# anshumang/gunrockINST

Measured on AMD Instinct MI355X. Metric: MTEPS (million traversed edges/sec) BFS R-MAT scale-24, higher is better.
Workload: dtype int32; 1 GPU; BFS idempotent direction-optimizing (traversal_mode 2), R-MAT scale-24 (a=.55 b=.2 c=.2 d=.05, 8 pairs/vertex mirrored, seed 0x6772): n=16777216, m=265395436 directed edges; sources: largest-degree + 64 seeded; search_depth_src0=7, max_degree=218420

## Files before the change

gunrockinst_amd/capi.py:

```python
import ctypes as C
import os
import subprocess

import numpy as np

_PKG = os.path.dirname(os.path.abspath(__file__))
LIB_PATH = os.environ.get("GUNROCK_LIB_PATH") or os.path.join(_PKG, "lib", "libgunrock.so")
_LIB = None

VTXID_INT = 0
SIZET_INT = 0
VALUE_INT, VALUE_UINT, VALUE_FLOAT = 0, 1, 2
SRC_MANUALLY, SRC_RANDOMIZE, SRC_LARGEST_DEGREE = 0, 1, 2

i32p = C.POINTER(C.c_int32)


class GunrockDataType(C.Structure):
    _fields_ = [("VTXID_TYPE", C.c_int), ("SIZET_TYPE", C.c_int), ("VALUE_TYPE", C.c_int)]


class GunrockGraph(C.Structure):
    _fields_ = [("num_nodes", C.c_size_t), ("num_edges", C.c_size_t),
                ("row_offsets", C.c_void_p), ("col_indices", C.c_void_p),
                ("col_offsets", C.c_void_p), ("row_indices", C.c_void_p),
                ("node_values", C.c_void_p), ("edge_values", C.c_void_p)]


class GunrockConfig(C.Structure):
    _fields_ = [("mark_pred", C.c_bool), ("idempotence", C.c_bool),
                ("src_node", C.c_int), ("device", C.c_int), ("max_iter", C.c_int),
                ("top_nodes", C.c_int), ("delta_factor", C.c_int),
                ("delta", C.c_float), ("error", C.c_float), ("queue_size", C.c_float),
                ("src_mode", C.c_int)]


def build_library(force=False):
    src_dir = os.path.join(_PKG, "csrc")
    if force:
        subprocess.check_call(["make", "-C", src_dir, "clean"])
    subprocess.check_call(["make", "-C", src_dir, "-j8", "-s"])
    return LIB_PATH


_SIGNATURES = {
    "gunrock_bfs_func": (None, [C.POINTER(GunrockGraph), C.POINTER(GunrockGraph), GunrockConfig, GunrockDataType]),
    "gunrock_bc_func": (None, [C.POINTER(GunrockGraph), C.POINTER(GunrockGraph), GunrockConfig, GunrockDataType]),
    "gunrock_cc_func": (None, [C.POINTER(GunrockGraph), C.POINTER(GunrockGraph), GunrockConfig, GunrockDataType]),
    "gunrock_sssp_func": (None, [C.POINTER(GunrockGraph), C.c_void_p, C.POINTER(GunrockGraph), GunrockConfig,
                                 GunrockDataType]),
    "gunrock_pr_func": (None, [C.POINTER(GunrockGraph), C.c_void_p, C.c_void_p, C.POINTER(GunrockGraph),
                               GunrockConfig, GunrockDataType]),
    "gunrock_topk_func": (None, [C.POINTER(GunrockGraph), C.c_void_p, C.c_void_p, C.c_void_p,
                                 C.POINTER(GunrockGraph), GunrockConfig, GunrockDataType]),
    "grx_graph_from_market": (C.c_int, [C.c_char_p, C.c_int, C.c_int, C.POINTER(C.c_void_p)]),
    "grx_graph_from_market_cached": (C.c_int, [C.c_char_p, C.c_int, C.c_int, C.POINTER(C.c_int), C.POINTER(C.c_void_p)]),
    "grx_graph_rmat_libc": (C.c_int, [C.c_int, C.c_int, C.c_int] + [C.c_double] * 4 + [C.POINTER(C.c_void_p)]),
    "grx_graph_rmat_seeded": (C.c_int, [C.c_int, C.c_longlong, C.c_uint64, C.c_int] + [C.c_double] * 4 +
                              [C.POINTER(C.c_void_p)]),
    "grx_graph_from_coo": (C.c_int, [C.c_int, C.c_longlong, i32p, i32p, i32p, C.POINTER(C.c_void_p)]),
    "grx_graph_from_csr": (C.c_int, [C.c_int, C.c_int, i32p, i32p, i32p, C.POINTER(C.c_void_p)]),
    "grx_graph_nodes": (C.c_int, [C.c_void_p]),
    "grx_graph_edges": (C.c_int, [C.c_void_p]),
    "grx_graph_row_offsets": (i32p, [C.c_void_p]),
    "grx_graph_col_indices": (i32p, [C.c_void_p]),
    "grx_graph_edge_values": (i32p, [C.c_void_p]),
    "grx_graph_highest_degree_node": (C.c_int, [C.c_void_p, i32p]),
    "grx_graph_average_degree": (C.c_int, [C.c_void_p]),
    "grx_random_node": (C.c_int, [C.c_int]),
    "grx_graph_free": (None, [C.c_void_p]),
    "grx_rmat_seeded_device": (C.c_int, [C.c_int, C.c_longlong, C.c_longlong, C.c_uint64] + [C.c_double] * 4 +
                               [C.c_void_p, C.c_void_p, C.c_void_p]),
    "grx_coo_to_csr_sort": (C.c_int, [C.POINTER(C.c_void_p), C.c_int, C.c_int, C.c_longlong, C.c_void_p, C.c_void_p, C.c_int,
                                      C.c_int, C.c_int, C.POINTER(C.c_longlong), C.c_void_p]),
    "grx_coo_to_csr_emit": (C.c_int, [C.c_void_p, C.c_void_p, C.c_void_p, C.c_void_p]),
    "grx_coo_to_csr_free": (None, [C.c_void_p]),
    "grx_bc_create": (C.c_int, [C.POINTER(C.c_void_p), C.c_int]),
    "grx_bc_init": (C.c_int, [C.c_void_p, C.c_int, C.c_int, C.c_void_p, C.c_void_p]),
    "grx_bc_init_device": (C.c_int, [C.c_void_p, C.c_int, C.c_int, C.c_void_p, C.c_void_p]),
    "grx_bc_run": (C.c_int, [C.c_void_p, C.c_int, C.c_int, C.c_double, C.POINTER(C.c_float)]),
    "grx_bc_extract": (C.c_int, [C.c_void_p, C.c_void_p, C.c_void_p, C.c_void_p]),
    "grx_bc_destroy": (None, [C.c_void_p]),
    "grx_bfs_create": (C.c_int, [C.POINTER(C.c_void_p), C.c_int, C.c_int, C.c_int, C.c_int]),
    "grx_bfs_init": (C.c_int, [C.c_void_p, C.c_int, C.c_int, i32p, i32p]),
    "grx_bfs_init_device": (C.c_int, [C.c_void_p, C.c_int, C.c_int, C.c_void_p, C.c_void_p]),
    "grx_bfs_set_inverse_graph": (C.c_int, [C.c_void_p, C.c_void_p, C.c_void_p, C.c_float, C.c_float]),
    "grx_bfs_auto_inverse": (C.c_int, [C.c_void_p, C.c_int, C.POINTER(C.c_int), C.POINTER(C.c_int), C.POINTER(C.c_float)]),
    "grx_bfs_set_tuning": (C.c_int, [C.c_void_p, C.c_float, C.c_float, C.c_float, C.c_int]),
    "grx_bfs_set_persistent_limit": (C.c_int, [C.c_void_p, C.c_int]),
    "grx_bfs_set_twc_limit": (C.c_int, [C.c_void_p, C.c_int]),
    "grx_bfs_set_binned_min_edges": (C.c_int, [C.c_void_p, C.c_longlong]),
    "grx_bfs_set_label_deferral": (C.c_int, [C.c_void_p, C.c_int, C.c_int]),
    "grx_bfs_set_option": (C.c_int, [C.c_void_p, C.c_char_p, C.c_double]),
    "grx_bfs_set_cooperative_launch": (C.c_int, [C.c_void_p, C.c_int]),
    "grx_bfs_set_head_pass": (C.c_int, [C.c_void_p, C.c_int, C.c_int]),
    "grx_bfs_reset": (C.c_int, [C.c_void_p, C.c_int, C.c_double]),
    "grx_bfs_enact": (C.c_int, [C.c_void_p, C.c_int, C.c_int, C.c_int, C.POINTER(C.c_float)]),
    "grx_bfs_stats": (C.c_int, [C.c_void_p, C.POINTER(C.c_longlong), C.POINTER(C.c_longlong),
                                C.POINTER(C.c_double), C.POINTER(C.c_longlong), C.POINTER(C.c_double)]),
    "grx_bfs_level_trace": (C.c_int, [C.c_void_p, C.c_int, C.POINTER(C.c_longlong), C.POINTER(C.c_longlong),
                                      C.POINTER(C.c_double), i32p]),
    "grx_bfs_extract": (C.c_int, [C.c_void_p, i32p, i32p]),
    "grx_bfs_device_results": (C.c_int, [C.c_void_p, C.POINTER(C.c_void_p), C.POINTER(C.c_void_p)]),
    "grx_bfs_mask_flushes": (C.c_int, [C.c_void_p, C.POINTER(C.c_longlong)]),
    "grx_bfs_relabel_info": (C.c_int, [C.c_void_p, C.POINTER(C.c_longlong), C.POINTER(C.c_longlong), C.POINTER(C.c_int),
                                       C.POINTER(C.c_float), C.POINTER(C.c_longlong)]),
    "grx_bfs_destroy": (None, [C.c_void_p]),
    "grx_cc_create": (C.c_int, [C.POINTER(C.c_void_p), C.c_int, C.c_int]),
    "grx_cc_init": (C.c_int, [C.c_void_p, C.c_int, C.c_int, i32p, i32p]),
    "grx_cc_init_device": (C.c_int, [C.c_void_p, C.c_int, C.c_int, C.c_void_p, C.c_void_p]),
    "grx_cc_reset": (C.c_int, [C.c_void_p]),
    "grx_cc_enact": (C.c_int, [C.c_void_p, C.c_int, C.POINTER(C.c_float)]),
    "grx_cc_stats": (C.c_int, [C.c_void_p, C.POINTER(C.c_longlong), C.POINTER(C.c_longlong), C.POINTER(C.c_longlong),
                               C.POINTER(C.c_double)]),
    "grx_cc_mirrored": (C.c_int, [C.c_void_p, C.POINTER(C.c_int)]),
    "grx_cc_sweep_edges": (C.c_int, [C.c_void_p, C.POINTER(C.c_longlong)]),
    "grx_cc_extract": (C.c_int, [C.c_void_p, i32p, C.POINTER(C.c_uint)]),
    "grx_cc_device_results": (C.c_int, [C.c_void_p, C.POINTER(C.c_void_p)]),
    "grx_cc_destroy": (None, [C.c_void_p]),
    "grx_mst_create": (C.c_int, [C.POINTER(C.c_void_p), C.c_int, C.c_int]),
    "grx_mst_init": (C.c_int, [C.c_void_p, C.c_int, C.c_int, i32p, i32p, i32p]),
    "grx_mst_init_device": (C.c_int, [C.c_void_p, C.c_int, C.c_int, C.c_void_p, C.c_void_p, C.c_void_p]),
    "grx_mst_reset": (C.c_int, [C.c_void_p]),
    "grx_mst_enact": (C.c_int, [C.c_void_p, C.c_int, C.POINTER(C.c_float)]),
    "grx_mst_stats": (C.c_int, [C.c_void_p, C.POINTER(C.c_longlong), C.POINTER(C.c_longlong), C.POINTER(C.c_longlong),
                                C.POINTER(C.c_double)]),
    "grx_mst_round_trace": (C.c_int, [C.c_void_p, C.c_int, C.POINTER(C.c_longlong), C.POINTER(C.c_double)]),
    "grx_mst_extract": (C.c_int, [C.c_void_p, i32p, C.POINTER(C.c_longlong), C.POINTER(C.c_int)]),
    "grx_mst_device_results": (C.c_int, [C.c_void_p, C.POINTER(C.c_void_p)]),
    "grx_mst_destroy": (None, [C.c_void_p]),
    "grx_mis_create": (C.c_int, [C.POINTER(C.c_void_p), C.c_int, C.c_int]),
    "grx_mis_init": (C.c_int, [C.c_void_p, C.c_int, C.c_int, i32p, i32p, i32p, C.c_uint]),
    "grx_mis_init_device": (C.c_int, [C.c_void_p, C.c_int, C.c_int, C.c_void_p, C.c_void_p, C.c_void_p, C.c_uint]),
    "grx_mis_set_tail": (C.c_int, [C.c_void_p, C.c_int]),
    "grx_mis_reset": (C.c_int, [C.c_void_p]),
    "grx_mis_enact": (C.c_int, [C.c_void_p, C.c_int, C.c_int, C.POINTER(C.c_float)]),
    "grx_mis_stats": (C.c_int, [C.c_void_p, C.POINTER(C.c_longlong), C.POINTER(C.c_longlong), C.POINTER(C.c_longlong),
                                C.POINTER(C.c_longlong), C.POINTER(C.c_longlong), C.POINTER(C.c_double)]),
    "grx_mis_round_trace": (C.c_int, [C.c_void_p, C.c_int, C.POINTER(C.c_longlong), C.POINTER(C.c_double)]),
    "grx_mis_extract": (C.c_int, [C.c_void_p, i32p, C.POINTER(C.c_longlong)]),
    "grx_mis_device_results": (C.c_int, [C.c_void_p, C.POINTER(C.c_void_p)]),
    "grx_mis_destroy": (None, [C.c_void_p]),
    "grx_tc_create": (C.c_int, [C.POINTER(C.c_void_p), C.c_int, C.c_int]),
    "grx_tc_init": (C.c_int, [C.c_void_p, C.c_int, C.c_int, i32p, i32p]),
    "grx_tc_init_device": (C.c_int, [C.c_void_p, C.c_int, C.c_int, C.c_void_p, C.c_void_p]),
    "grx_tc_set_option": (C.c_int, [C.c_void_p, C.c_char_p, C.c_double]),
    "grx_tc_reset": (C.c_int, [C.c_void_p]),
    "grx_tc_enact": (C.c_int, [C.c_void_p, C.c_int, C.POINTER(C.c_float)]),
    "grx_tc_stats": (C.c_int, [C.c_void_p, C.POINTER(C.c_longlong), C.POINTER(C.c_longlong), C.POINTER(C.c_longlong),
                               C.POINTER(C.c_longlong), C.POINTER(C.c_longlong), C.POINTER(C.c_double), C.POINTER(C.c_double)]),
    "grx_tc_extract": (C.c_int, [C.c_void_p, C.POINTER(C.c_longlong), C.POINTER(C.c_longlong)]),
    "grx_tc_clustering": (C.c_int, [C.c_void_p, C.POINTER(C.c_double), C.POINTER(C.c_double)]),
    "grx_tc_device_results": (C.c_int, [C.c_void_p, C.POINTER(C.c_void_p), C.POINTER(C.c_void_p)]),
    "grx_tc_destroy": (None, [C.c_void_p]),
    "grx_kcore_create": (C.c_int, [C.POINTER(C.c_void_p), C.c_int, C.c_int]),
    "grx_kcore_init": (C.c_int, [C.c_void_p, C.c_int, C.c_int, i32p, i32p]),
    "grx_kcore_init_device": (C.c_int, [C.c_void_p, C.c_int, C.c_int, C.c_void_p, C.c_void_p]),
    "grx_kcore_set_option": (C.c_int, [C.c_void_p, C.c_char_p, C.c_double]),
    "grx_kcore_reset": (C.c_int, [C.c_void_p]),
    "grx_kcore_enact": (C.c_int, [C.c_void_p, C.c_int, C.c_int, C.POINTER(C.c_float)]),
    "grx_kcore_stats": (C.c_int, [C.c_void_p] + [C.POINTER(C.c_longlong)] * 8 + [C.POINTER(C.c_double)] * 2),
    "grx_kcore_level_trace": (C.c_int, [C.c_void_p, C.c_int, i32p, C.POINTER(C.c_longlong), C.POINTER(C.c_double)]),
    "grx_kcore_extract": (C.c_int, [C.c_void_p, i32p, C.POINTER(C.c_int)]),
    "grx_kcore_shells": (C.c_int, [C.c_void_p, C.c_int, C.POINTER(C.c_longlong)]),
    "grx_kcore_members": (C.c_int, [C.c_void_p, C.c_int, C.POINTER(C.c_ubyte), C.POINTER(C.c_longlong), C.POINTER(C.c_longlong)]),
    "grx_kcore_device_results": (C.c_int, [C.c_void_p, C.POINTER(C.c_void_p), C.POINTER(C.c_void_p)]),
    "grx_kcore_destroy": (None, [C.c_void_p]),
    "grx_truss_create": (C.c_int, [C.POINTER(C.c_void_p), C.c_int, C.c_int]),
    "grx_truss_init": (C.c_int, [C.c_void_p, C.c_int, C.c_int, i32p, i32p]),
    "grx_truss_init_device": (C.c_int, [C.c_void_p, C.c_int, C.c_int, C.c_void_p, C.c_void_p]),
    "grx_truss_set_option": (C.c_int, [C.c_void_p, C.c_char_p, C.c_double]),
    "grx_truss_reset": (C.c_int, [C.c_void_p]),
    "grx_truss_enact": (C.c_int, [C.c_void_p, C.c_int, C.c_int, C.POINTER(C.c_float)]),
    "grx_truss_stats": (C.c_int, [C.c_void_p] + [C.POINTER(C.c_longlong)] * 10 + [C.POINTER(C.c_double)] * 3),
    "grx_truss_level_trace": (C.c_int, [C.c_void_p, C.c_int, i32p, C.POINTER(C.c_longlong), C.POINTER(C.c_double)]),
    "grx_truss_edges": (C.c_int, [C.c_void_p, i32p, i32p]),
    "grx_truss_support": (C.c_int, [C.c_void_p, i32p, C.POINTER(C.c_longlong)]),
    "grx_truss_extract": (C.c_int, [C.c_void_p, i32p, C.POINTER(C.c_int)]),
    "grx_truss_classes": (C.c_int, [C.c_void_p, C.c_int, C.POINTER(C.c_longlong)]),
    "grx_truss_members": (C.c_int, [C.c_void_p, C.c_int, C.POINTER(C.c_ubyte), C.POINTER(C.c_longlong), C.POINTER(C.c_longlong)]),
    "grx_truss_vertex_truss": (C.c_int, [C.c_void_p, i32p]),
    "grx_truss_device_results": (C.c_int, [C.c_void_p] + [C.POINTER(C.c_void_p)] * 4),
    "grx_truss_destroy": (None, [C.c_void_p]),
    "grx_sssp_create": (C.c_int, [C.POINTER(C.c_void_p), C.c_int, C.c_int, C.c_int]),
    "grx_sssp_init": (C.c_int, [C.c_void_p, C.c_int, C.c_int, i32p, i32p, C.POINTER(C.c_uint32), C.c_int]),
    "grx_sssp_init_device": (C.c_int, [C.c_void_p, C.c_int, C.c_int, C.c_void_p, C.c_void_p, C.c_void_p, C.c_float]),
    "grx_sssp_set_inverse_graph": (C.c_int, [C.c_void_p, C.c_void_p, C.c_void_p, C.c_void_p, C.c_longlong]),
# ... 234 lines not shown

    def set_inverse_graph(self, d_inv_row_offsets=None, d_inv_col_indices=None, alpha=0.0, beta=0.0):
        _check(lib().grx_bfs_set_inverse_graph(self._h, C.c_void_p(d_inv_row_offsets), C.c_void_p(d_inv_col_indices),
                                               alpha, beta), "BFSProblem::SetInverseGraph")
        return self

    def auto_inverse(self, build_if_directed=True):
        on, made, ms = C.c_int(), C.c_int(), C.c_float()
        _check(lib().grx_bfs_auto_inverse(self._h, int(bool(build_if_directed)), C.byref(on), C.byref(made), C.byref(ms)),
               "grx_bfs_auto_inverse")
        return bool(on.value), bool(made.value), float(ms.value)

    def set_tuning(self, alpha=0.0, beta=0.0, lite_factor=-1.0, tail_edge_limit=-1):
        _check(lib().grx_bfs_set_tuning(self._h, alpha, beta, lite_factor, tail_edge_limit), "grx_bfs_set_tuning")
        return self

    def set_head_pass(self, min_edges=-1, max_edges=-1):
        _check(lib().grx_bfs_set_head_pass(self._h, int(min_edges), int(max_edges)), "grx_bfs_set_head_pass")
        return self

    def set_option(self, name, value):
        _check(lib().grx_bfs_set_option(self._h, name.encode(), float(value)), "grx_bfs_set_option(%s)" % name)
        return self

    def set_label_deferral(self, enabled=-1, mask_limit=0):
        _check(lib().grx_bfs_set_label_deferral(self._h, int(enabled), int(mask_limit)), "grx_bfs_set_label_deferral")
        return self

    def set_binned_min_edges(self, min_edges):
        _check(lib().grx_bfs_set_binned_min_edges(self._h, int(min_edges)), "grx_bfs_set_binned_min_edges")
        return self

    def set_cooperative_launch(self, on=True):
        _check(lib().grx_bfs_set_cooperative_launch(self._h, int(bool(on))), "grx_bfs_set_cooperative_launch")
        return self

    def set_persistent_limit(self, edge_limit):
        _check(lib().grx_bfs_set_persistent_limit(self._h, int(edge_limit)), "grx_bfs_set_persistent_limit")
        return self

    def set_twc_limit(self, edge_limit):
        _check(lib().grx_bfs_set_twc_limit(self._h, int(edge_limit)), "grx_bfs_set_twc_limit")
        return self

    def reset(self, src, queue_sizing=1.0):
        _check(lib().grx_bfs_reset(self._h, int(src), float(queue_sizing)), "BFSProblem::Reset")

    def enact(self, src, max_grid_size=0, traversal_mode=0):
        return self._timed(lib().grx_bfs_enact, "BFSEnactor::Enact", int(src), max_grid_size, traversal_mode)

    def stats(self):
        q, d, l = C.c_longlong(), C.c_longlong(), C.c_longlong()
        duty, kms = C.c_double(), C.c_double()
        _check(lib().grx_bfs_stats(self._h, C.byref(q), C.byref(d), C.byref(duty), C.byref(l), C.byref(kms)),
               "BFSEnactor::GetStatistics")
        return {"total_queued": q.value, "search_depth": d.value, "avg_duty": duty.value,
                "kernel_launches": l.value, "kernel_ms": kms.value}

    def level_trace(self, max_levels=4096):
        fr = (C.c_longlong * max_levels)()
        ed = (C.c_longlong * max_levels)()
        ms = (C.c_double * max_levels)()
        kd = (C.c_int32 * max_levels)()
        n = lib().grx_bfs_level_trace(self._h, max_levels, fr, ed, ms, kd)
        n = min(max(n, 0), max_levels)
        return [{"frontier": fr[i], "edges": ed[i], "ms": ms[i], "kind": kd[i]} for i in range(n)]

    def extract(self):
        labels = np.empty(max(self.nodes, 1), dtype=np.int32)
        preds = np.empty(max(self.nodes, 1), dtype=np.int32) if self.mark_pred else None
        _check(lib().grx_bfs_extract(self._h, _p(labels), None if preds is None else _p(preds)), "BFSProblem::Extract")
        return labels[:self.nodes], (None if preds is None else preds[:self.nodes])

    def device_results(self):
        dl, dp = C.c_void_p(), C.c_void_p()
        _check(lib().grx_bfs_device_results(self._h, C.byref(dl), C.byref(dp)), "grx_bfs_device_results")
        return dl.value, dp.value

    def mask_flushes(self):
        v = C.c_longlong()
        _check(lib().grx_bfs_mask_flushes(self._h, C.byref(v)), "grx_bfs_mask_flushes")
        return v.value

    def relabel_info(self):
        h, we, t, ms, b = C.c_longlong(), C.c_longlong(), C.c_int(), C.c_float(), C.c_longlong()
        _check(lib().grx_bfs_relabel_info(self._h, C.byref(h), C.byref(we), C.byref(t), C.byref(ms), C.byref(b)),
               "grx_bfs_relabel_info")
        return {"hubs": h.value, "with_edges": we.value, "threshold": t.value, "build_ms": ms.value, "bytes": b.value}


def _graph_struct(nodes, row_offsets, col_indices, edge_values=None):
    g = GunrockGraph()
    g.num_nodes = nodes
    g.num_edges = col_indices.shape[0]
    g.row_offsets = row_offsets.ctypes.data
    g.col_indices = col_indices.ctypes.data
    g.edge_values = None if edge_values is None else edge_values.ctypes.data
    return g


def _take_node_values(gout, nodes, dtype):
    ptr = gout.node_values
    if not ptr:
        raise RuntimeError("gunrockinst_amd: the call produced no node_values")
    arr = np.ctypeslib.as_array(C.cast(ptr, C.POINTER(C.c_int32)), shape=(max(nodes, 1),))[:nodes].copy()
    C.CDLL(None).free(C.c_void_p(ptr))
    return arr.view(dtype)


def gunrock_bfs(nodes, row_offsets, col_indices, src=0, mark_pred=False, idempotence=False, queue_size=1.0,
                src_mode=SRC_MANUALLY, device=0):
    ro, ci = _csr_arrays(row_offsets, col_indices)
    gin = _graph_struct(nodes, ro, ci)
    gout = GunrockGraph()
    cfg = GunrockConfig()
    cfg.mark_pred, cfg.idempotence = mark_pred, idempotence
    cfg.src_node, cfg.device, cfg.queue_size, cfg.src_mode = src, device, queue_size, src_mode
    dt = GunrockDataType(VTXID_INT, SIZET_INT, VALUE_INT)
    lib().gunrock_bfs_func(C.byref(gout), C.byref(gin), cfg, dt)
    return _take_node_values(gout, nodes, np.int32)


class CcProblem(_Handle):

    _destroy = "grx_cc_destroy"

    def __init__(self, instrument=False, device=0):
        self._create("grx_cc_create", int(instrument), device)
        self.nodes = 0

    def init(self, nodes, row_offsets, col_indices):
        ro, ci = _csr_arrays(row_offsets, col_indices)
        self.nodes = int(nodes)
        _check(lib().grx_cc_init(self._h, nodes, ci.shape[0], _p(ro), _p(ci)), "CCProblem::Init")
        return self

    def init_device(self, nodes, edges, d_row_offsets, d_col_indices):
        self.nodes = int(nodes)
        _check(lib().grx_cc_init_device(self._h, nodes, edges, C.c_void_p(d_row_offsets), C.c_void_p(d_col_indices)),
               "CCProblem::Init(device)")
        return self

    def reset(self):
        _check(lib().grx_cc_reset(self._h), "CCProblem::Reset")

    def enact(self, max_grid_size=0):
        return self._timed(lib().grx_cc_enact, "CCEnactor::Enact", max_grid_size)

    def stats(self):
        es, vs, l = C.c_longlong(), C.c_longlong(), C.c_longlong()
        k = C.c_double()
        _check(lib().grx_cc_stats(self._h, C.byref(es), C.byref(vs), C.byref(l), C.byref(k)), "grx_cc_stats")
        mir = C.c_int()
        _check(lib().grx_cc_mirrored(self._h, C.byref(mir)), "grx_cc_mirrored")
        se = C.c_longlong()
        _check(lib().grx_cc_sweep_edges(self._h, C.byref(se)), "grx_cc_sweep_edges")
        return {"edge_sweeps": es.value, "vertex_sweeps": vs.value, "kernel_launches": l.value, "kernel_ms": k.value,
                "mirrored": bool(mir.value), "sweep_edges": se.value}

    def extract(self):
        ids = np.empty(max(self.nodes, 1), dtype=np.int32)
        nc = C.c_uint()
        _check(lib().grx_cc_extract(self._h, _p(ids), C.byref(nc)), "CCProblem::Extract")
        return ids[:self.nodes], int(nc.value)

    def device_results(self):
# ... 794 lines not shown
```

gunrockinst_amd/csrc/gunrock/app/bfs/bfs_enactor.hpp:

```cpp
#pragma once

#include <hip/hip_runtime.h>
#include <cstdlib>

#include <gunrock/app/bfs/bfs_functor.hpp>
#include <gunrock/app/bfs/bfs_problem.hpp>
#include <gunrock/app/enactor_base.hpp>
#include <gunrock/oprtr/advance/bottom_up.hpp>
#include <gunrock/oprtr/advance/kernel.hpp>
#include <gunrock/oprtr/advance/twc.hpp>
#include <gunrock/util/context.hpp>

namespace gunrock {
namespace app {
namespace bfs {

template <bool INSTRUMENT>
class BFSEnactor : public EnactorBase {
   public:
    explicit BFSEnactor(bool DEBUG = false) : EnactorBase(VERTEX_FRONTIERS, DEBUG) {}
    ~BFSEnactor() override {}

    void GetKernelStatistics(long long &launches, double &kernel_ms)
    {
// ... 222 lines not shown
                hipLaunchKernelGGL((oprtr::advance::BottomUpKernel<BU_THREADS, 8, 32, BFSProblem, L, false>),
                                   dim3(static_cast<unsigned>(grid)), dim3(BU_THREADS), 0, stream, bargs, *ds, lookup);
            return util::GRError("BottomUpKernel launch failed", __FILE__, __LINE__);
        };
        const int chain_len = (dobfs && problem->chain_sweeps > 0)
            ? (problem->chain_sweeps < oprtr::advance::kChainMax ? problem->chain_sweeps : oprtr::advance::kChainMax) : 0;
        work_progress.publish_sets = chain_len > 0 ? chain_len + 1 : 1;
        oprtr::advance::SweepRule sweep_rule;
        sweep_rule.with_in_edges = problem->with_in_edges;
        sweep_rule.nodes = problem->nodes;
        sweep_rule.beta = problem->beta;
        sweep_rule.emit_factor = problem->emit_queue_factor;
        sweep_rule.sparse_div = problem->sparse_sweep_div;
        auto run_sweep_chain = [&](long long first_in) -> hipError_t {
            typedef oprtr::advance::BitmapLookup<VertexId> L;
            hipError_t rc = hipSuccess;
            const long long it0 = iteration;
            const long long base_total = enactor_stats.total_queued;
            int masks[oprtr::advance::kChainMax + 1];
            masks[0] = cur_mask;
            int queued = 0;
            const long long bu_steps = ((static_cast<long long>(problem->nodes) + 63) / 64 + oprtr::advance::kBottomUpStepWords - 1) / oprtr::advance::kBottomUpStepWords;
            long long grid = (bu_steps + (BU_THREADS / 64) - 1) / (BU_THREADS / 64);
            const bool walk_queue = problem->walk_queue != 0;
            const long long cap = max_grid_size > 0 ? max_grid_size
                : walk_queue ? util::ResidentGrid(oprtr::advance::BottomUpAutoKernel<BU_THREADS, 8, 32, BFSProblem, L, true>, BU_THREADS)
                             : util::ResidentGrid(oprtr::advance::BottomUpAutoKernel<BU_THREADS, 8, 32, BFSProblem, L, false>, BU_THREADS);
            if (grid > cap) grid = cap;
            if (grid < 1) grid = 1;
            const long long chunks = ((static_cast<long long>(problem->nodes) + 63) / 64 + oprtr::advance::kSparseChunkWords - 1) / oprtr::advance::kSparseChunkWords;
            long long sparse_grid = (chunks + (BU_THREADS / 64) - 1) / (BU_THREADS / 64);
            if (sparse_grid < 1) sparse_grid = 1;
            long long emit_grid = sparse_grid < cu_count * 4 ? sparse_grid : cu_count * 4;
            for (int k = 1; k <= chain_len; ++k) {
                bool got = false;
                if ((rc = problem->TryAcquireMask(stream, masks[k], masks, k, got))) return rc;
                if (!got) break;
                oprtr::advance::BottomUpArgs<VertexId, SizeT> bargs;
                bargs.nodes = problem->nodes;
                bargs.d_inv_row_offsets = ds->d_inv_row_offsets;
                bargs.d_inv_column_indices = ds->d_inv_column_indices;
                bargs.d_inv_heads = ds->d_inv_heads;
                L lookup{ds->d_frontier_mask[masks[k - 1]]};
                bargs.d_frontier_out = reinterpret_cast<unsigned long long *>(ds->d_frontier_mask[masks[k]]);
                bargs.d_visited = reinterpret_cast<unsigned long long *>(ds->d_visited_mask);
                const long long level = it0 + k - 1;
                bargs.d_tail_out = work_progress.d_tail + ((level + 1) & 3);
                bargs.d_tail_clear = work_progress.d_tail + ((level + 2) & 3);
                bargs.d_wide = work_progress.d_wide + static_cast<size_t>(k) * util::WorkProgress::kWideSetWords;
                bargs.head_skip = 0;
                bargs.heads_only = 0;
                bargs.d_never = reinterpret_cast<const unsigned long long *>(ds->d_never_mask);
                bargs.d_head_base = ds->d_head_base;
                bargs.d_duty = INSTRUMENT ? DutySlot() : nullptr;
                bargs.queue_out = gs->frontier_queues[selector];
                bargs.d_fwd_row_offsets = gs->d_row_offsets;
                bargs.d_queue_tail = work_progress.d_tail + ((level + 1) & 3);
                bargs.d_queue_invalid = reinterpret_cast<int *>(work_progress.AuxTail());
                bargs.d_overflow = work_progress.d_overflow;
                oprtr::advance::SweepChain chain;
                chain.d_sets = work_progress.d_wide;
                chain.base_total = base_total;
                chain.first_in = first_in;
                chain.rule = sweep_rule;
                chain.index = k;
                chain.first_may_switch = 0;
                chain.d_log = work_progress.d_chain_log;
                typename BFSProblem::DataSlice level_slice = *ds;
                level_slice.iteration = static_cast<VertexId>(level);
                if (walk_queue)
                    hipLaunchKernelGGL((oprtr::advance::BottomUpAutoKernel<BU_THREADS, 8, 32, BFSProblem, L, true>), dim3(static_cast<unsigned>(grid)),
                                       dim3(BU_THREADS), 0, stream, bargs, level_slice, lookup, chain, static_cast<unsigned>(sparse_grid),
                                       static_cast<unsigned>(emit_grid));
                else
                    hipLaunchKernelGGL((oprtr::advance::BottomUpAutoKernel<BU_THREADS, 8, 32, BFSProblem, L, false>), dim3(static_cast<unsigned>(grid)),
                                       dim3(BU_THREADS), 0, stream, bargs, level_slice, lookup, chain, static_cast<unsigned>(sparse_grid),
                                       static_cast<unsigned>(emit_grid));
                if ((rc = util::GRError("BottomUpAutoKernel launch failed", __FILE__, __LINE__))) return rc;
                queued = k;
            }
            if (queued == 0) return util::GRError(hipErrorInvalidValue, "BFSEnactor: no frontier bitmap for a bottom-up sweep", __FILE__, __LINE__);
            const bool closing_queued = problem->chain_closing && problem->persistent_edge_limit > 0;
            int *d_gate = work_progress.d_chain_log + 8;
            bool emit_queued = false;
            if (closing_queued) {
                oprtr::advance::PersistentArgs<VertexId, SizeT> p;
                p.t.queue[0] = gs->frontier_queues[0];
                p.t.queue[1] = gs->frontier_queues[1];
                p.t.selector = selector;
                p.t.first_iteration = it0;
                p.t.d_tail = work_progress.d_tail;
                p.t.max_levels = kTailMaxLevels;
                p.t.d_levels_done = work_progress.LevelsDone();
                p.t.d_level_sums = work_progress.d_sums;
                p.t.d_row_offsets = gs->d_row_offsets;
                p.t.d_column_indices = gs->d_column_indices;
                p.t.d_overflow = work_progress.d_overflow;
                p.t.edge_limit = static_cast<SizeT>(static_cast<long long>(problem->persistent_edge_limit) * 4);
                p.barrier.d_counter = work_progress.BarrierCounter();
                p.barrier.d_timeout = work_progress.BarrierTimeout();
                p.solo_edges = problem->tail_edge_limit / 4;
                p.unexplored_edges = unexplored_edges;
                p.switch_factor = 0.0;
                oprtr::advance::SweepChain chain;
                chain.d_sets = work_progress.d_wide;
                chain.base_total = base_total;
                chain.first_in = first_in;
                chain.rule = sweep_rule;
                chain.index = queued;
                chain.first_may_switch = 0;
                chain.d_log = work_progress.d_chain_log;
                if ((rc = oprtr::advance::LaunchChainedPersistentLevels<PersistentPolicy, BFSProblem, BfsFunctor>(
                         p, *ds, cu_count, chain, queued, it0, reinterpret_cast<const int *>(work_progress.AuxTail()), d_gate, stream)))
                    return rc;
                if (deferring && problem->speculative_emit && problem->level_masks.count + queued <= app::bfs::kLevelMasks) {
                    VertexId labels[oprtr::advance::kChainMax];
                    for (int k = 1; k <= queued; ++k) labels[k - 1] = static_cast<VertexId>(it0 + k);
                    if ((rc = problem->EmitLabelsGated(stream, masks + 1, labels, queued, d_gate))) return rc;
                    emit_queued = true;
                }
            }
            if (INSTRUMENT && (rc = InstrumentEnd(stream))) return rc;
            if ((rc = work_progress.Sync(stream))) return rc;
            long long total = base_total;
            int ran = 0, last_action = oprtr::advance::kSweepStop;
            long long next_in = 0;
            for (int k = 1; k <= queued + 1; ++k) {
                const long long in_k = (k == 1 && first_in >= 0) ? first_in
                    : static_cast<long long>(util::TailCount(k == 1 ? work_progress.box->wide : work_progress.box->wide_set[k - 1]));
                next_in = in_k;
                if (k > queued) break;
                const int action = sweep_rule.Decide(in_k, total + in_k, k > 1);
                if (action != work_progress.box->chain_log[k])
                    return util::GRError(hipErrorUnknown, "BFSEnactor: host and device disagree about a chained sweep", __FILE__, __LINE__);
                if (action <= oprtr::advance::kSweepSwitch) break;
                total += in_k;
                ran = k;
                last_action = action;
                if (deferring) problem->KeepMask(masks[k], static_cast<VertexId>(it0 + k));
            }
            enactor_stats.total_queued = total;
            iteration = it0 + ran;
            cur_mask = masks[ran];
            queue_length = static_cast<unsigned>(next_in);
            queue_edges = 0;
            queue_emitted = ran > 0 && last_action == oprtr::advance::kSweepSparseEmit;
            out_slot_clean = ran > 0 && !queue_emitted;
            if (queue_emitted && work_progress.h_tail[util::WorkProgress::kAux] != 0) {
                queue_emitted = false;
                if ((rc = work_progress.ClearAux(stream))) return rc;
            }
            if (INSTRUMENT) InstrumentCollect(static_cast<long long>(first_in >= 0 ? first_in : 0), 0, 1);
            if (closing_queued && ran >= 1 && queue_emitted && queue_length > 0 &&
                sweep_rule.Decide(next_in, total + next_in, true) == oprtr::advance::kSweepSwitch) {
                if (work_progress.HostBarrierTimedOut())
                    return util::GRError(hipErrorLaunchTimeOut, "BFSEnactor persistent levels kernel: grid barrier timed out", __FILE__, __LINE__);
                const int done = work_progress.HostLevelsDone();
                iteration += done;
                selector ^= (done & 1);
                queue_length = util::TailCount(work_progress.h_tail[iteration & 3]);
                queue_edges = util::TailEdges(work_progress.h_tail[iteration & 3]);
                enactor_stats.total_queued += static_cast<long long>(work_progress.h_sums[0]);
                enactor_stats.total_edges_queued += static_cast<long long>(work_progress.h_sums[1]);
                unexplored_edges -= static_cast<long long>(work_progress.h_sums[1]);
                bottom_up = false;
                queue_emitted = false;
                out_slot_clean = false;
                snapshot_valid = false;
                if (emit_queued) problem->emit_current = queue_length == 0;
            }
            return rc;
        };
        auto launch_count_only = [&](oprtr::advance::AdvanceArgs<VertexId, SizeT> args) -> hipError_t {
            ds->lite = 1;
            if (INSTRUMENT && !args.d_duty) args.d_duty = DutySlot();
            args.d_tail_out = nullptr;
            hipError_t rc = oprtr::advance::LaunchKernel<AdvancePolicy, BFSProblem, BfsFunctor, true, true>(args, *ds, max_grid_size, stream,
                                                                                                              oprtr::advance::V2V);
            ds->lite = 0;
            return rc;
        };
        auto launch_fresh_pass = [&](const unsigned long long *d_before, const unsigned long long *d_merge, int out_mask) -> hipError_t {
            const long long words64 = (static_cast<long long>(problem->nodes) + 63) / 64;
            long long fgrid = ((words64 + 15) / 16 + 3) / 4;
            if (fgrid > cu_count * 4) fgrid = cu_count * 4;
            hipLaunchKernelGGL((oprtr::advance::FreshToBitmapKernel<VertexId>), dim3(static_cast<unsigned>(fgrid)), dim3(256), 0, stream,
                               ds->d_fresh, static_cast<long long>(problem->nodes), reinterpret_cast<unsigned long long *>(ds->d_visited_mask),
                               d_before, reinterpret_cast<unsigned long long *>(ds->d_frontier_mask[out_mask]),
                               deferring ? static_cast<VertexId *>(nullptr) : ds->d_labels, static_cast<VertexId>(iteration + 1), work_progress.d_tail + ((iteration + 1) & 3), work_progress.d_wide,
                               d_merge, work_progress.d_tail + ((iteration + 2) & 3));
            if (deferring) problem->KeepMask(out_mask, static_cast<VertexId>(iteration + 1));
            return util::GRError("FreshToBitmapKernel launch failed", __FILE__, __LINE__);
        };
        auto queue_to_mask = [&](int out_mask) -> hipError_t {
            hipError_t rc;
            if (!snapshot_valid) {
                if ((rc = util::GRError(hipMemsetAsync(ds->d_frontier_mask[out_mask], 0, mask_bytes, stream),
                                        "BFSEnactor hipMemsetAsync frontier mask failed", __FILE__, __LINE__)))
                    return rc;
                hipLaunchKernelGGL((oprtr::advance::QueueToBitmapKernel<VertexId, SizeT>), dim3(conv_grid), dim3(256), 0, stream,
                                   gs->frontier_queues[selector].v, static_cast<SizeT>(queue_length), ds->d_frontier_mask[out_mask]);
                return util::GRError("QueueToBitmapKernel launch failed", __FILE__, __LINE__);
            }
            const long long words64 = static_cast<long long>(problem->MaskWords()) / 2;
            hipLaunchKernelGGL(oprtr::advance::BitmapDiffKernel, dim3(conv_grid), dim3(256), 0, stream,
                               reinterpret_cast<const unsigned long long *>(ds->d_visited_mask),
                               reinterpret_cast<const unsigned long long *>(ds->d_snapshot),
                               reinterpret_cast<unsigned long long *>(ds->d_frontier_mask[out_mask]), words64);
            return util::GRError("BitmapDiffKernel launch failed", __FILE__, __LINE__);
        };
        while (queue_length > 0) {
            const unsigned in_len = queue_length, in_edges = queue_edges;
            bool binned_level = false;
            if (INSTRUMENT && (retval = InstrumentBegin(stream))) break;

            if (dobfs && !bottom_up && !force_bottom_up && problem->head_pass_min_edges != 0 &&
                static_cast<long long>(queue_edges) >= problem->HeadPassMin() &&
                static_cast<long long>(queue_edges) <= problem->HeadPassMax() &&
                queue_edges > static_cast<unsigned>(problem->tail_edge_limit) &&
                static_cast<double>(queue_edges) * problem->alpha * problem->lite_factor > static_cast<double>(unexplored_edges)) {
                enactor_stats.total_queued += queue_length;
                enactor_stats.total_edges_queued += queue_edges;
                unexplored_edges -= queue_edges;
                ds->iteration = static_cast<VertexId>(iteration);
                int front_mask = 0, heads_mask = 0, out_mask = 0;
                if ((retval = problem->AcquireMask(stream, front_mask))) break;
                if ((retval = queue_to_mask(front_mask))) break;
                if ((retval = problem->AcquireMask(stream, heads_mask, front_mask))) break;
                if ((retval = launch_bottom_up(front_mask, heads_mask, 1))) break;
                oprtr::advance::AdvanceArgs<VertexId, SizeT> args;
                args.in = gs->frontier_queues[selector];
                args.out = gs->frontier_queues[selector ^ 1];
                args.in_len = static_cast<SizeT>(queue_length);
                args.in_edges = static_cast<SizeT>(queue_edges);
                args.d_row_offsets = gs->d_row_offsets;
                args.d_column_indices = gs->d_column_indices;
                args.d_tail_out = nullptr;
                args.d_tail_clear = nullptr;
                args.d_overflow = work_progress.d_overflow;
                if ((retval = launch_count_only(args))) break;
                if ((retval = problem->AcquireMask(stream, out_mask, front_mask, heads_mask))) break;
                if ((retval = launch_fresh_pass(reinterpret_cast<const unsigned long long *>(ds->d_visited_mask),
                                                reinterpret_cast<const unsigned long long *>(ds->d_frontier_mask[heads_mask]), out_mask)))
                    break;
                cur_mask = out_mask;
                snapshot_valid = false;
                ++iteration;
                if (chain_len > 0) {
                    if (INSTRUMENT) {
                        if ((retval = InstrumentEnd(stream))) break;
                        if ((retval = util::GRError(hipStreamSynchronize(stream), "BFSEnactor instrument sync failed", __FILE__, __LINE__))) break;
                        InstrumentCollect(in_len, in_edges, 6);
// ... 216 lines not shown
```

gunrockinst_amd/csrc/gunrock/app/bfs/bfs_problem.hpp:

```cpp
#pragma once

#include <hip/hip_runtime.h>

#include <gunrock/app/problem_base.hpp>
#include <gunrock/graphio/device_csr.hpp>
#include <gunrock/graphio/relabel.hpp>
#include <gunrock/oprtr/advance/binned.hpp>
#include <gunrock/oprtr/advance/bottom_up.hpp>
#include <gunrock/util/memset_kernel.hpp>

namespace gunrock {
namespace app {
namespace bfs {

template <typename SizeT>
__global__ void NoInEdgeMaskKernel(const SizeT *d_inv_row_offsets, long long nodes, long long words64, unsigned long long *d_mask)
{
    const unsigned lane = threadIdx.x & 63;
    const long long wave0 = (static_cast<long long>(blockIdx.x) * blockDim.x + threadIdx.x) / 64;
    const long long nwaves = static_cast<long long>(gridDim.x) * blockDim.x / 64;
    for (long long w = wave0; w < words64; w += nwaves) {
        const long long v = w * 64 + lane;
        const bool none = v < nodes && d_inv_row_offsets[v + 1] == d_inv_row_offsets[v];
        const unsigned long long m = __ballot(none);
// ... 186 lines not shown
        if (j == 1) l = lab[1];
        if (j == 2) l = lab[2];
        if (j == 3) l = lab[3];
        if ((keep >> j) & 1u) l = d_work_labels[x1 + j];
        out[b] = l;
        if (PRED) {
            const VertexId p = d_work_preds[x1 + j];
            pout[b] = p >= 0 ? d_old_of_new[p] : p;
        }
        ++j;
    }
}

template <typename VertexId, int KMAX, bool PRED>
__global__ __launch_bounds__(256) void TranslateLabelsKernel(LevelMaskList<VertexId> levels, const unsigned long long *d_visited,
                                                             graphio::RelabelView map, long long nodes, VertexId caller_src,
                                                             const VertexId *d_work_labels, const VertexId *d_work_preds,
                                                             const VertexId *d_old_of_new, VertexId *d_labels, VertexId *d_preds)
{
    typedef __attribute__((ext_vector_type(4))) int V4;
    int valid = KMAX;
    if (levels.d_gate) {
        if (levels.d_gate[0] == 0) return;
        valid = levels.chain_first + levels.d_gate[1];
    }
    const bool hubs = map.hubs > 0;
    const long long quads = (nodes + 3) / 4;
    const long long stride = static_cast<long long>(gridDim.x) * blockDim.x;
    for (long long q = static_cast<long long>(blockIdx.x) * blockDim.x + threadIdx.x; q < quads; q += stride) {
        const long long v0 = q * 4;
        const long long w = v0 >> 6;
        const int sh = static_cast<int>(v0 & 63);
        const unsigned long long edge = map.d_edge[w];
        const unsigned long long hub = hubs ? map.d_hub[w] : 0ull;
        const long long b1 = map.d_base1[w];
        const long long b0 = hubs ? map.d_base0[w] : 0ll;
        const unsigned long long low = (1ull << sh) - 1ull;
        const unsigned h4 = static_cast<unsigned>(hub >> sh) & 0xFu, e4 = static_cast<unsigned>(edge >> sh) & 0xFu;
        int out[4] = {-1, -1, -1, -1};
        int pout[4] = {-2, -2, -2, -2};
        if (e4)
            TranslateTier<VertexId, KMAX, PRED>(levels, valid, d_visited, e4, map.hubs + b1 + __popcll(edge & low), d_work_labels, d_work_preds,
                                                d_old_of_new, out, pout);
        if (h4)
            TranslateTier<VertexId, KMAX, PRED>(levels, valid, d_visited, h4, b0 + __popcll(hub & low), d_work_labels, d_work_preds,
                                                d_old_of_new, out, pout);
#pragma unroll
        for (int b = 0; b < 4; ++b)
            if (caller_src == v0 + b && !(((h4 | e4) >> b) & 1u)) {
                out[b] = 0;
                pout[b] = -1;
            }
        if (v0 + 3 < nodes) {
            *reinterpret_cast<V4 *>(d_labels + v0) = V4{out[0], out[1], out[2], out[3]};
            if (PRED) *reinterpret_cast<V4 *>(d_preds + v0) = V4{pout[0], pout[1], pout[2], pout[3]};
        } else {
            for (int b = 0; b < 4 && v0 + b < nodes; ++b) {
                d_labels[v0 + b] = out[b];
                if (PRED) d_preds[v0 + b] = pout[b];
            }
        }
    }
}

constexpr int kLabelTileWords = 64;
constexpr int kLabelSpan = kLabelTileWords + 2;
static_assert(kLabelSpan <= 128 && kLabelTileWords % 16 == 0, "phase 1 maps one tier to each half of the workgroup");
constexpr unsigned kCodeWorkLabel = 13u;
static_assert(kLevelMasks < kCodeWorkLabel && kCodeWorkLabel < 16u, "four code planes");

typedef __attribute__((ext_vector_type(4))) unsigned LabelPlanes;

__device__ __forceinline__ void TiledWindow(const LabelPlanes *planes, const unsigned char *spread, unsigned t4, unsigned x, unsigned first_half,
                                            unsigned (&e)[4])
{
    const unsigned j = (x >> 5) - first_half;
    const LabelPlanes lo = planes[j], hi = planes[j + 1];
    const unsigned row = t4 << 4;
#pragma unroll
    for (int p = 0; p < 4; ++p)
        e[p] |= spread[row | (__builtin_amdgcn_alignbit(hi[p], lo[p], x) & 0xFu)];
}

template <typename VertexId, bool RELABEL, bool PRED>
__global__ __launch_bounds__(256) void TiledLabelsKernel(LevelMaskList<VertexId> levels, const unsigned long long *d_visited,
                                                         const unsigned long long *d_never, graphio::RelabelView map, long long nodes,
                                                         VertexId src, const VertexId *d_work_labels, const VertexId *d_work_preds,
                                                         const VertexId *d_old_of_new, VertexId *d_labels, VertexId *d_preds)
{
    typedef __attribute__((ext_vector_type(4))) int V4;
    __shared__ LabelPlanes planes[2][2 * kLabelSpan];
    __shared__ uint2 s_tier[2][2 * kLabelTileWords];
    __shared__ int table[16];
    __shared__ unsigned char spread[256];
    const int t = threadIdx.x;
    const long long words = (nodes + 63) / 64;
    const long long w0 = static_cast<long long>(blockIdx.x) * kLabelTileWords;
    const bool hubs = RELABEL && map.hubs > 0;
    long long xw1 = w0, xwh = 0;
    if (RELABEL) {
        xw1 = (map.hubs + map.d_base1[w0]) >> 6;
        if (hubs) xwh = map.d_base0[w0] >> 6;
    }
    int valid = levels.count;
    if (levels.d_gate) {
        const int go = levels.d_gate[0], filled = levels.d_gate[1];
        if (go == 0) return;
        valid = levels.chain_first + filled;
    }
    if (t < 16) table[t] = (t >= 1 && t <= kLevelMasks) ? levels.label[t - 1] : -1;
    if (RELABEL) {
        unsigned dealt = 0u;
        for (int b = 0, r = 0; b < 4; ++b)
            if ((t >> (4 + b)) & 1) {
                dealt |= ((static_cast<unsigned>(t) >> r) & 1u) << b;
                ++r;
            }
        spread[t] = static_cast<unsigned char>(dealt);
    }
    unsigned long long tile_edge = 0ull, tile_hub = 0ull;
    unsigned tile_base1 = 0u, tile_base0 = 0u;
    if (RELABEL && t < kLabelTileWords && w0 + t < words) {
        tile_edge = map.d_edge[w0 + t];
        tile_base1 = map.d_base1[w0 + t];
        if (hubs) {
            tile_hub = map.d_hub[w0 + t];
            tile_base0 = map.d_base0[w0 + t];
        }
    }
    const int tier = t >> 7, col = t & 127;
    if (col < kLabelSpan && (tier == 0 || hubs)) {
        const long long word = (tier ? xwh : xw1) + col;
        const bool live = col < (RELABEL ? kLabelTileWords + 1 : kLabelTileWords) && word < words;
        const long long at = live ? word : 0;
        unsigned long long m[kLevelMasks];
#pragma unroll
        for (int k = 0; k < kLevelMasks; ++k) m[k] = levels.mask[k][at];
        const unsigned long long vis = d_visited[at];
        const unsigned long long nev = (!RELABEL && d_never) ? d_never[at] : 0ull;
        unsigned long long pl[4] = {0ull, 0ull, 0ull, 0ull}, later = 0ull;
#pragma unroll
        for (int k = kLevelMasks - 1; k >= 0; --k) {
            const unsigned long long own = (k < valid ? m[k] : 0ull) & ~later;
            later |= own;
#pragma unroll
            for (int p = 0; p < 4; ++p)
                if (((k + 1) >> p) & 1) pl[p] |= own;
        }
        const unsigned long long kept = vis & ~nev & ~later;
#pragma unroll
        for (int p = 0; p < 4; ++p) {
            if ((kCodeWorkLabel >> p) & 1u) pl[p] |= kept;
            if (!live) pl[p] = 0ull;
        }
        planes[tier][2 * col] = LabelPlanes{static_cast<unsigned>(pl[0]), static_cast<unsigned>(pl[1]), static_cast<unsigned>(pl[2]), static_cast<unsigned>(pl[3])};
        planes[tier][2 * col + 1] = LabelPlanes{static_cast<unsigned>(pl[0] >> 32), static_cast<unsigned>(pl[1] >> 32), static_cast<unsigned>(pl[2] >> 32),
                                                static_cast<unsigned>(pl[3] >> 32)};
    }
    if (RELABEL && t < kLabelTileWords) {
        const unsigned e_lo = static_cast<unsigned>(tile_edge), h_lo = static_cast<unsigned>(tile_hub);
        const unsigned x1 = static_cast<unsigned>(map.hubs) + tile_base1;
        s_tier[0][2 * t] = make_uint2(e_lo, x1);
        s_tier[0][2 * t + 1] = make_uint2(static_cast<unsigned>(tile_edge >> 32), x1 + __popc(e_lo));
        s_tier[1][2 * t] = make_uint2(h_lo, tile_base0);
        s_tier[1][2 * t + 1] = make_uint2(static_cast<unsigned>(tile_hub >> 32), tile_base0 + __popc(h_lo));
    }
    __syncthreads();
    const int sh = (t & 15) * 4;
    const int half = sh >> 5, s5 = sh & 31;
    const unsigned below = (1u << s5) - 1u;
    const unsigned first1 = static_cast<unsigned>(xw1) * 2u, firsth = static_cast<unsigned>(xwh) * 2u;
    constexpr int kSteps = kLabelTileWords / 16;
    int outs[kSteps][4], pouts[PRED ? kSteps : 1][4];
#pragma unroll
    for (int i = 0; i < kSteps; ++i) {
        const int wi = i * 16 + (t >> 4);
        const long long w = w0 + wi;
        if (w >= words) continue;
        const long long v0 = w * 64 + sh;
        int(&out)[4] = outs[i];
        unsigned e[4] = {0u, 0u, 0u, 0u};
        unsigned e4 = 0u, h4 = 0u, x1 = 0u, xh = 0u;
        if (RELABEL) {
            const uint2 m1 = s_tier[0][2 * wi + half];
            e4 = (m1.x >> s5) & 0xFu;
            x1 = m1.y + __popc(m1.x & below);
            TiledWindow(planes[0], spread, e4, x1, first1, e);
            if (hubs) {
                const uint2 mh = s_tier[1][2 * wi + half];
                h4 = (mh.x >> s5) & 0xFu;
                xh = mh.y + __popc(mh.x & below);
                TiledWindow(planes[1], spread, h4, xh, firsth, e);
            }
        } else {
            const LabelPlanes c = planes[0][2 * wi + half];
#pragma unroll
            for (int p = 0; p < 4; ++p) e[p] = (c[p] >> s5) & 0xFu;
        }
        const unsigned packed = e[0] | (e[1] << 6) | (e[2] << 12) | (e[3] << 18);
#pragma unroll
        for (int b = 0; b < 4; ++b) {
            const unsigned at = (__umul24(packed & (0x041041u << b), 0x8421u) >> (13 + b)) & 0x3Cu;
            out[b] = *reinterpret_cast<const int *>(reinterpret_cast<const char *>(table) + at);
        }
        int pout[4] = {-2, -2, -2, -2};
        const unsigned work = e[0] & ~e[1] & e[2] & e[3];
        const bool src_here = static_cast<unsigned long long>(static_cast<long long>(src) - v0) < 4ull;
        if (work || src_here || PRED) {
#pragma unroll
            for (int b = 0; b < 4; ++b) {
                if (RELABEL) {
                    const unsigned lower = (1u << b) - 1u;
                    const bool in1 = (e4 >> b) & 1u, in0 = (h4 >> b) & 1u;
                    const unsigned x = in1 ? x1 + __popc(e4 & lower) : xh + __popc(h4 & lower);
                    if ((work >> b) & 1u) out[b] = d_work_labels[x];
                    if (PRED && (in1 || in0)) {
                        const VertexId p = d_work_preds[x];
                        pout[b] = p >= 0 ? d_old_of_new[p] : p;
                    }
                    if (src == v0 + b && !in1 && !in0) {
                        out[b] = 0;
                        pout[b] = -1;
                    }
                } else if ((((work >> b) & 1u) || src == v0 + b) && v0 + b < nodes) {
                    out[b] = d_work_labels[v0 + b];
                }
            }
        }
        if (PRED)
#pragma unroll
            for (int b = 0; b < 4; ++b) pouts[PRED ? i : 0][b] = pout[b];
    }
#pragma unroll
    for (int i = 0; i < kSteps; ++i) {
        const long long w = w0 + i * 16 + (t >> 4);
        if (w >= words) continue;
        const long long v0 = w * 64 + sh;
        const int(&out)[4] = outs[i];
        const int(&pout)[4] = pouts[PRED ? i : 0];
        if (v0 + 3 < nodes) {
            __builtin_nontemporal_store(V4{out[0], out[1], out[2], out[3]}, reinterpret_cast<V4 *>(d_labels + v0));
            if (PRED) __builtin_nontemporal_store(V4{pout[0], pout[1], pout[2], pout[3]}, reinterpret_cast<V4 *>(d_preds + v0));
        } else {
            for (int b = 0; b < 4 && v0 + b < nodes; ++b) {
                d_labels[v0 + b] = out[b];
                if (PRED) d_preds[v0 + b] = pout[b];
            }
        }
    }
}

template <typename VertexId, typename SizeT>
struct SearchGraph {
    SizeT *d_row_offsets = nullptr;
    VertexId *d_column_indices = nullptr;
    const SizeT *d_inv_row_offsets = nullptr;
    const VertexId *d_inv_column_indices = nullptr;
    unsigned *d_never_mask = nullptr;
    unsigned *d_head_base = nullptr;
    int2 *d_inv_heads = nullptr;
    long long with_in_edges = 0;

    void Release()
    {
        if (d_never_mask) util::GRError(hipFree(d_never_mask), "SearchGraph hipFree d_never_mask failed", __FILE__, __LINE__);
        if (d_head_base) util::GRError(hipFree(d_head_base), "SearchGraph hipFree d_head_base failed", __FILE__, __LINE__);
        if (d_inv_heads) util::GRError(hipFree(d_inv_heads), "SearchGraph hipFree d_inv_heads failed", __FILE__, __LINE__);
        d_never_mask = nullptr;
        d_head_base = nullptr;
        d_inv_heads = nullptr;
    }

    hipError_t Build(long long nodes, long long mask_words, hipStream_t stream)
    {
        hipError_t retval = hipSuccess;
        if (!d_never_mask)
            GR_CHECK(hipMalloc(&d_never_mask, sizeof(unsigned) * static_cast<size_t>(mask_words + 2)), "SearchGraph hipMalloc d_never_mask failed");
        if (!d_inv_heads)
            GR_CHECK(hipMalloc(&d_inv_heads, sizeof(int2) * static_cast<size_t>(nodes > 0 ? nodes : 1)), "SearchGraph hipMalloc d_inv_heads failed");
        const long long words64 = mask_words / 2 + 1;
        long long grid = (words64 + 3) / 4;
        if (grid > 2048) grid = 2048;
        hipLaunchKernelGGL((NoInEdgeMaskKernel<SizeT>), dim3(static_cast<unsigned>(grid)), dim3(256), 0, stream, d_inv_row_offsets, nodes, words64,
                           reinterpret_cast<unsigned long long *>(d_never_mask));
        GR_CHECK(hipGetLastError(), "NoInEdgeMaskKernel launch failed");
        if (!d_head_base)
            GR_CHECK(hipMalloc(&d_head_base, sizeof(unsigned) * static_cast<size_t>(words64 + 1)), "SearchGraph hipMalloc d_head_base failed");
        unsigned *d_counts = nullptr;
        unsigned long long *d_scan_sums = nullptr;
        GR_CHECK(hipMalloc(&d_counts, sizeof(unsigned) * static_cast<size_t>(words64 + 1)), "SearchGraph hipMalloc failed");
        GR_CHECK(hipMalloc(&d_scan_sums, sizeof(unsigned long long) * static_cast<size_t>(graphio::ScanScratchWords(words64))), "SearchGraph hipMalloc failed");
        hipLaunchKernelGGL(WithInEdgesCountKernel, dim3(static_cast<unsigned>((words64 + 255) / 256)), dim3(256), 0, stream,
                           reinterpret_cast<const unsigned long long *>(d_never_mask), nodes, words64, d_counts);
        GR_CHECK(hipGetLastError(), "WithInEdgesCountKernel launch failed");
        GR_CHECK(graphio::DeviceExclusiveScan<unsigned>(d_counts, d_head_base, words64, d_scan_sums, stream), "SearchGraph head-base scan failed");
        GR_CHECK(hipStreamSynchronize(stream), "NoInEdgeMaskKernel failed");
        {
            unsigned last_base = 0, last_count = 0;
            GR_CHECK(hipMemcpy(&last_base, d_head_base + (words64 - 1), sizeof(unsigned), hipMemcpyDeviceToHost), "SearchGraph read failed");
            GR_CHECK(hipMemcpy(&last_count, d_counts + (words64 - 1), sizeof(unsigned), hipMemcpyDeviceToHost), "SearchGraph read failed");
            with_in_edges = static_cast<long long>(last_base) + last_count;
        }
        GR_CHECK(hipFree(d_counts), "SearchGraph hipFree failed");
        GR_CHECK(hipFree(d_scan_sums), "SearchGraph hipFree failed");
        if (nodes > 0) {
            long long hgrid = (nodes + 3) / 4;
            if (hgrid > 8192) hgrid = 8192;
            hipLaunchKernelGGL((oprtr::advance::BuildHeadsKernel<VertexId, SizeT>), dim3(static_cast<unsigned>(hgrid)), dim3(256), 0, stream,
                               d_inv_row_offsets, d_inv_column_indices, nodes, d_inv_heads, d_inv_row_offsets,
                               reinterpret_cast<const unsigned long long *>(d_never_mask), d_head_base);
            GR_CHECK(hipGetLastError(), "BuildHeadsKernel launch failed");
            GR_CHECK(hipStreamSynchronize(stream), "BuildHeadsKernel failed");
        }
        return retval;
    }
};

template <typename _VertexId, typename _SizeT, typename _Value, bool _MARK_PREDECESSORS,
          bool _ENABLE_IDEMPOTENCE, bool _USE_DOUBLE_BUFFER>
struct BFSProblem : ProblemBase<_VertexId, _SizeT, _Value, _USE_DOUBLE_BUFFER> {
    typedef ProblemBase<_VertexId, _SizeT, _Value, _USE_DOUBLE_BUFFER> Base;
    typedef _VertexId VertexId;
    typedef _SizeT SizeT;
    typedef _Value Value;
    static constexpr bool MARK_PREDECESSORS = _MARK_PREDECESSORS;
    static constexpr bool ENABLE_IDEMPOTENCE = _ENABLE_IDEMPOTENCE;

    struct DataSlice {
        VertexId *d_labels = nullptr;
        VertexId *d_preds = nullptr;
        unsigned *d_visited_mask = nullptr;
        VertexId iteration = 0;
        int lite = 0;
        int defer_labels = 0;
        unsigned char *d_fresh = nullptr;
        unsigned *d_frontier_mask[kLevelMasks] = {};
        unsigned *d_snapshot = nullptr;
        unsigned *d_never_mask = nullptr;
        unsigned *d_head_base = nullptr;
        int2 *d_inv_heads = nullptr;
        const SizeT *d_inv_row_offsets = nullptr;
        const VertexId *d_inv_column_indices = nullptr;
    };

    bool direction_optimizing = false;
    float alpha = 10.0f;
    float beta = 4000.0f;
    int twc_edge_limit = 8192;
    float lite_factor = 700.0f;
    int head_pass_min_edges = -1;
    int head_pass_max_edges = -1;
    long long with_in_edges = 0;
    int sparse_sweep_div = 6;
    float emit_queue_factor = 128.0f;
    bool chain_closing = true;
    bool speculative_emit = true;
    int chain_sweeps = 4;
    long long HeadPassMin() const { return head_pass_min_edges >= 0 ? head_pass_min_edges : static_cast<long long>(this->edges) / 30 + 1; }
    long long HeadPassMax() const
    {
        if (head_pass_max_edges > 0) return head_pass_max_edges;
        if (head_pass_max_edges == 0) return 1ll << 40;
        return static_cast<long long>(static_cast<double>(this->edges) / 7.8);
    }
    long long binned_min_edges = 1ll << 23;
    oprtr::advance::BinPoolStorage<VertexId> bin_pool;
    bool cooperative_launch = false;
    int persistent_edge_limit = 1 << 20;
    int tail_edge_limit = 8192;

    DataSlice **data_slices = nullptr;
    DataSlice **d_data_slices = nullptr;

    BFSProblem() {}

    ~BFSProblem() override
    {
        if (data_slices && active != 0) UseNumbering(0);
        if (data_slices) {
            DataSlice *ds = data_slices[0];
            if (ds) {
                if (d_out_labels) util::GRError(hipFree(d_out_labels), "BFSProblem hipFree d_labels failed", __FILE__, __LINE__);
                if (d_out_preds) util::GRError(hipFree(d_out_preds), "BFSProblem hipFree d_preds failed", __FILE__, __LINE__);
                if (d_work_labels) util::GRError(hipFree(d_work_labels), "BFSProblem hipFree work labels failed", __FILE__, __LINE__);
                if (d_work_preds) util::GRError(hipFree(d_work_preds), "BFSProblem hipFree work preds failed", __FILE__, __LINE__);
                if (ds->d_visited_mask) util::GRError(hipFree(ds->d_visited_mask), "BFSProblem hipFree d_visited_mask failed", __FILE__, __LINE__);
                for (int i = 0; i < kLevelMasks; ++i)
                    if (ds->d_frontier_mask[i]) util::GRError(hipFree(ds->d_frontier_mask[i]), "BFSProblem hipFree d_frontier_mask failed", __FILE__, __LINE__);
                if (ds->d_snapshot) util::GRError(hipFree(ds->d_snapshot), "BFSProblem hipFree d_snapshot failed", __FILE__, __LINE__);
                if (ds->d_fresh) util::GRError(hipFree(ds->d_fresh), "BFSProblem hipFree d_fresh failed", __FILE__, __LINE__);
                delete ds;
            }
            delete[] data_slices;
        }
        for (int k = 0; k < 2; ++k) numbering[k].Release();
        relabelled.Release();
        if (h_src_box) util::GRError(hipHostFree(h_src_box), "BFSProblem hipHostFree failed", __FILE__, __LINE__);
        bin_pool.Release();
    }

    SizeT MaskWords() const { return ((this->nodes + 63) / 64) * 2; }

    SearchGraph<VertexId, SizeT> numbering[2];
    graphio::RelabelledCsr relabelled;
    int relabel = -1;
    long long relabel_min_nodes = 1ll << 23;
    long long relabel_hubs = 0;
    bool build_relabelled = false;
    int active = 0;
    bool translate_pending = false;
    VertexId caller_source = -1;
    VertexId *d_out_labels = nullptr, *d_out_preds = nullptr;
    VertexId *d_work_labels = nullptr, *d_work_preds = nullptr;

    hipError_t BuildRelabelled(long long hubs)
    {
        hipError_t retval = hipSuccess;
        hipStream_t stream = this->graph_slices[0]->stream;
        if (!direction_optimizing || numbering[0].d_inv_row_offsets != numbering[0].d_row_offsets)
            return util::GRError(hipErrorInvalidValue, "BFSProblem: the relabelled copy needs a symmetric graph (InverseIsSelf)", __FILE__, __LINE__);
        GR_CHECK(hipStreamSynchronize(stream), "BFSProblem sync failed");
        if (active == 1) UseNumbering(0);
        numbering[1].Release();
        GR_CHECK(relabelled.Build(this->nodes, this->edges, numbering[0].d_row_offsets, numbering[0].d_column_indices, hubs < 0 ? 0 : hubs,
                                  MARK_PREDECESSORS, stream),
                 "BFSProblem relabel build failed");
        numbering[1].d_row_offsets = relabelled.d_row_offsets;
        numbering[1].d_column_indices = relabelled.d_cols;
        numbering[1].d_inv_row_offsets = relabelled.d_row_offsets;
        numbering[1].d_inv_column_indices = relabelled.d_cols;
        GR_CHECK(numbering[1].Build(this->nodes, MaskWords(), stream), "BFSProblem relabelled static state failed");
        const size_t n = static_cast<size_t>(this->nodes > 0 ? this->nodes : 1);
        if (!d_work_labels) GR_CHECK(hipMalloc(&d_work_labels, sizeof(VertexId) * n), "BFSProblem hipMalloc work labels failed");
        if (MARK_PREDECESSORS && !d_work_preds) GR_CHECK(hipMalloc(&d_work_preds, sizeof(VertexId) * n), "BFSProblem hipMalloc work preds failed");
        relabel_hubs = hubs;
        return retval;
    }
    bool HasRelabelled() const { return relabelled.Ready() && numbering[1].d_never_mask != nullptr; }
    bool RelabelActive() const
    {
        return HasRelabelled() && (relabel > 0 || (relabel < 0 && static_cast<long long>(this->nodes) >= relabel_min_nodes));
    }
    VertexId SearchId(VertexId v) const { return (active == 1 && v >= 0 && v < this->nodes) ? static_cast<VertexId>(relabelled.NewId(v)) : v; }

    void UseNumbering(int k)
    {
        DataSlice *ds = data_slices[0];
        GraphSlice<VertexId, SizeT, Value> *gs = this->graph_slices[0];
        active = k;
        const SearchGraph<VertexId, SizeT> &g = numbering[k];
        gs->d_row_offsets = g.d_row_offsets;
        gs->d_column_indices = g.d_column_indices;
        ds->d_inv_row_offsets = g.d_inv_row_offsets;
        ds->d_inv_column_indices = g.d_inv_column_indices;
        ds->d_never_mask = g.d_never_mask;
        ds->d_head_base = g.d_head_base;
        ds->d_inv_heads = g.d_inv_heads;
        with_in_edges = g.with_in_edges;
        ds->d_labels = k == 1 ? d_work_labels : d_out_labels;
        ds->d_preds = k == 1 ? d_work_preds : d_out_preds;
    }

    hipError_t SetInverseGraph(const SizeT *d_inv_row_offsets, const VertexId *d_inv_column_indices,
                               float alpha_ = 0.0f, float beta_ = 0.0f)
    {
        hipError_t retval = hipSuccess;
        DataSlice *ds = data_slices[0];
        if (active != 0) UseNumbering(0);
        relabelled.Release();
        numbering[1].Release();
        numbering[0].d_row_offsets = this->graph_slices[0]->d_row_offsets;
        numbering[0].d_column_indices = this->graph_slices[0]->d_column_indices;
        numbering[0].d_inv_row_offsets = d_inv_row_offsets;
        numbering[0].d_inv_column_indices = d_inv_column_indices;
        for (int i = 0; i < kLevelMasks; ++i)
            if (!ds->d_frontier_mask[i])
                GR_CHECK(hipMalloc(&ds->d_frontier_mask[i], sizeof(unsigned) * static_cast<size_t>(MaskWords() + 2)),
                         "BFSProblem hipMalloc d_frontier_mask failed");
        if (!ds->d_snapshot)
            GR_CHECK(hipMalloc(&ds->d_snapshot, sizeof(unsigned) * static_cast<size_t>(MaskWords() + 2)), "BFSProblem hipMalloc d_snapshot failed");
        if (!ds->d_fresh) {
            const size_t bytes = (static_cast<size_t>(this->nodes) + 1023) / 1024 * 1024 + 1024;
            GR_CHECK(hipMalloc(&ds->d_fresh, bytes), "BFSProblem hipMalloc d_fresh failed");
            GR_CHECK(hipMemset(ds->d_fresh, 0, bytes), "BFSProblem hipMemset d_fresh failed");
            GR_CHECK(hipDeviceSynchronize(), "BFSProblem sync failed");
        }
        GR_CHECK(numbering[0].Build(static_cast<long long>(this->nodes), MaskWords(), this->graph_slices[0]->stream),
                 "BFSProblem static search state failed");
        UseNumbering(0);

        if (alpha_ > 0) alpha = alpha_;
        if (beta_ > 0) beta = beta_;
        direction_optimizing = true;
        return retval;
    }
    hipError_t EnsureBinned(int workgroups, int *d_overflow)
    {
        hipError_t retval = hipSuccess;
        DataSlice *ds = data_slices[0];
        if (!bin_pool.Ready() || bin_pool.workgroups < workgroups)
            GR_CHECK(bin_pool.Allocate(static_cast<long long>(this->edges), workgroups, MARK_PREDECESSORS, d_overflow),
                     "BFSProblem bin pool allocation failed");
        if (!ds->d_fresh) {
            const size_t bytes = (static_cast<size_t>(this->nodes) + 1023) / 1024 * 1024 + 1024;
            GR_CHECK(hipMalloc(&ds->d_fresh, bytes), "BFSProblem hipMalloc d_fresh failed");
            GR_CHECK(hipMemset(ds->d_fresh, 0, bytes), "BFSProblem hipMemset d_fresh failed");
            GR_CHECK(hipDeviceSynchronize(), "BFSProblem sync failed");
        }
        if (!ds->d_frontier_mask[0])
            GR_CHECK(hipMalloc(&ds->d_frontier_mask[0], sizeof(unsigned) * static_cast<size_t>(MaskWords() + 2)),
                     "BFSProblem hipMalloc d_frontier_mask failed");
        return retval;
    }

    hipError_t InverseIsSelf(float alpha_ = 0.0f, float beta_ = 0.0f)
    {
        hipError_t retval = hipSuccess;
        if (active != 0) UseNumbering(0);
        GR_CHECK(SetInverseGraph(this->graph_slices[0]->d_row_offsets, this->graph_slices[0]->d_column_indices, alpha_, beta_),
                 "BFSProblem SetInverseGraph failed");
        if (build_relabelled && this->nodes > 0 && BuildRelabelled(relabel_hubs) != hipSuccess) {
            hipGetLastError();
            relabelled.Release();
            numbering[1].Release();
            if (active != 0) UseNumbering(0);
        }
        return retval;
    }

    hipError_t AllocData()
    {
        hipError_t retval = hipSuccess;
        data_slices = new DataSlice *[1];
        data_slices[0] = new DataSlice();
        DataSlice *ds = data_slices[0];
        const size_t n = static_cast<size_t>(this->nodes > 0 ? this->nodes : 1);
        GR_CHECK(hipMalloc(&ds->d_labels, sizeof(VertexId) * n), "BFSProblem hipMalloc d_labels failed");
        if (MARK_PREDECESSORS)
            GR_CHECK(hipMalloc(&ds->d_preds, sizeof(VertexId) * n), "BFSProblem hipMalloc d_preds failed");
        d_out_labels = ds->d_labels;
        d_out_preds = ds->d_preds;
        GR_CHECK(hipMalloc(&ds->d_visited_mask, sizeof(unsigned) * static_cast<size_t>(MaskWords() + 2)),
                 "BFSProblem hipMalloc d_visited_mask failed");
        return retval;
    }

    hipError_t Init(bool stream_from_host, const Csr<VertexId, Value, SizeT> &graph, int num_gpus = 1)
    {
        hipError_t retval = hipSuccess;
        if ((retval = Base::Init(stream_from_host, graph, num_gpus))) return retval;
        return AllocData();
    }

    hipError_t InitFromDevice(SizeT nodes, SizeT edges, SizeT *d_row_offsets, VertexId *d_column_indices)
    {
        hipError_t retval = hipSuccess;
        if ((retval = Base::InitFromDevice(nodes, edges, d_row_offsets, d_column_indices))) return retval;
        return AllocData();
    }

    hipError_t Reset(VertexId src, FrontierType frontier_type, double queue_sizing)
    {
        hipError_t retval = hipSuccess;
        if ((retval = Base::Reset(frontier_type, queue_sizing))) return retval;
        GraphSlice<VertexId, SizeT, Value> *gs = this->graph_slices[0];
        DataSlice *ds = data_slices[0];
        hipStream_t stream = gs->stream;
        if (!h_src_box) {
            GR_CHECK(hipHostMalloc(reinterpret_cast<void **>(&h_src_box), sizeof(SourceBox), hipHostMallocMapped), "BFSProblem hipHostMalloc failed");
            h_src_box->seq = 0;
        }
        if (direction_optimizing) UseNumbering(RelabelActive() ? 1 : 0);
// ... 152 lines not shown
                                   d_work_labels, d_work_preds, relabelled.d_old_of_new, d_out_labels, d_out_preds);
                translate_pending = false;
            } else {
                hipLaunchKernelGGL((TiledLabelsKernel<VertexId, false, false>), tg, b, 0, stream, list, vis, nev, graphio::RelabelView(), n, src,
                                   ds->d_labels, nullptr, nullptr, ds->d_labels, nullptr);
            }
            level_masks.count = 0;
            return util::GRError(hipGetLastError(), "TiledLabelsKernel launch failed", __FILE__, __LINE__);
        }
        if (FULL && active == 1) {
            const graphio::RelabelView map = relabelled.View();
            const VertexId csrc = (caller_source >= 0 && caller_source < this->nodes) ? caller_source : static_cast<VertexId>(-1);
            const VertexId *o2n = relabelled.d_old_of_new;
#define GRX_TRANSLATE_CASE(K) case K: hipLaunchKernelGGL((TranslateLabelsKernel<VertexId, K, MARK_PREDECESSORS>), g, b, 0, stream, list, vis, map, n, csrc, \
                                                          d_work_labels, d_work_preds, o2n, d_out_labels, d_out_preds); break;
            switch (kmax) {
                GRX_TRANSLATE_CASE(0) GRX_TRANSLATE_CASE(1) GRX_TRANSLATE_CASE(2) GRX_TRANSLATE_CASE(3) GRX_TRANSLATE_CASE(4) GRX_TRANSLATE_CASE(5)
                GRX_TRANSLATE_CASE(6) GRX_TRANSLATE_CASE(7) GRX_TRANSLATE_CASE(8)
                default: hipLaunchKernelGGL((TranslateLabelsKernel<VertexId, kLevelMasks, MARK_PREDECESSORS>), g, b, 0, stream, list, vis, map, n, csrc,
                                            d_work_labels, d_work_preds, o2n, d_out_labels, d_out_preds);
            }
#undef GRX_TRANSLATE_CASE
            level_masks.count = 0;
            translate_pending = false;
            return util::GRError(hipGetLastError(), "TranslateLabelsKernel launch failed", __FILE__, __LINE__);
        }
#define GRX_EMIT_CASE(K) case K: hipLaunchKernelGGL((EmitLabelsKernel<VertexId, FULL, K>), g, b, 0, stream, list, vis, nev, n, src, ds->d_labels); break;
        switch (kmax) {
            GRX_EMIT_CASE(0) GRX_EMIT_CASE(1) GRX_EMIT_CASE(2) GRX_EMIT_CASE(3) GRX_EMIT_CASE(4) GRX_EMIT_CASE(5) GRX_EMIT_CASE(6) GRX_EMIT_CASE(7)
            GRX_EMIT_CASE(8)
            default: hipLaunchKernelGGL((EmitLabelsKernel<VertexId, FULL, kLevelMasks>), g, b, 0, stream, list, vis, nev, n, src, ds->d_labels);
        }
#undef GRX_EMIT_CASE
        level_masks.count = 0;
        return util::GRError(hipGetLastError(), "EmitLabelsKernel launch failed", __FILE__, __LINE__);
    }
    long long mask_flushes = 0;
    hipError_t FlushLevelMasks(hipStream_t stream)
    {
        if (level_masks.count == 0) return hipSuccess;
        ++mask_flushes;
        return LaunchEmit<false>(stream, static_cast<VertexId>(-1));
    }
    hipError_t FinishSearch(hipStream_t stream)
    {
        if (labels_deferred) return EmitLabels(stream);
        if (!translate_pending) return hipSuccess;
        level_masks.count = 0;
        return LaunchEmit<true>(stream, source);
    }
    hipError_t EmitLabels(hipStream_t stream)
    {
        if (!labels_deferred) return hipSuccess;
        labels_deferred = false;
        if (emit_current) {
            emit_current = false;
            level_masks.count = 0;
            return hipSuccess;
        }
        return LaunchEmit<true>(stream, (source >= 0 && source < this->nodes) ? source : static_cast<VertexId>(-1));
    }
    hipError_t EmitLabelsGated(hipStream_t stream, const int *chain_masks, const VertexId *chain_labels, int chain_count, const int *d_gate)
    {
        if (!labels_deferred || !speculative_emit) return hipSuccess;
        if (level_masks.count + chain_count > kLevelMasks) return hipSuccess;
        const LevelMaskList<VertexId> keep = level_masks;
        level_masks.chain_first = level_masks.count;
        for (int k = 0; k < chain_count; ++k) KeepMask(chain_masks[k], chain_labels[k]);
        level_masks.d_gate = d_gate;
        const hipError_t rc = LaunchEmit<true>(stream, (source >= 0 && source < this->nodes) ? source : static_cast<VertexId>(-1));
        level_masks = keep;
        return rc;
    }
    hipError_t EmitLabelsSpeculative(hipStream_t stream)
    {
        if (!labels_deferred || !speculative_emit) return hipSuccess;
        const LevelMaskList<VertexId> keep = level_masks;
        const hipError_t rc = LaunchEmit<true>(stream, (source >= 0 && source < this->nodes) ? source : static_cast<VertexId>(-1));
        level_masks = keep;
        emit_current = true;
        return rc;
    }

    util::WorkProgress *arm_progress = nullptr;
    util::WorkProgress *armed_progress = nullptr;

    VertexId source = -1;
    SizeT src_row[2] = {0, 0};
    struct SourceBox {
        unsigned long long seq;
        SizeT row[2];
    };
    SourceBox *h_src_box = nullptr;
    unsigned long long reset_seq = 0;
    bool src_row_pending = false;
};

}
}
}
```

gunrockinst_amd/csrc/gunrock/oprtr/advance/kernel.hpp:

```cpp
#pragma once

#include <hip/hip_runtime.h>
#include <cstdlib>
#include <climits>
#include <limits>
#include <type_traits>

#include <gunrock/oprtr/advance/binned.hpp>
#include <gunrock/oprtr/advance/functor_hooks.hpp>
#include <gunrock/oprtr/advance/sweep_chain.hpp>
#include <gunrock/oprtr/frontier_writer.hpp>
#include <gunrock/util/device_intrinsics.hpp>
#include <gunrock/util/error_utils.hpp>
#include <gunrock/util/frontier.hpp>
#include <gunrock/util/kernel_runtime_stats.hpp>

namespace gunrock {
namespace oprtr {
namespace advance {

enum MODE { TWC_FORWARD, TWC_BACKWARD, LB_BACKWARD, LB };
enum TYPE { V2V, V2E, E2V, E2E };
enum REDUCE_OP { NONE, PLUS, MINUS, MULTIPLIES, MODULUS, BIT_OR, BIT_AND, BIT_XOR, MAXIMUM, MINIMUM };
enum REDUCE_TYPE { EMPTY, VERTEX, EDGE };

template <int _THREADS, int _ITEMS_PER_THREAD, int _MIN_BLOCKS_PER_CU, MODE _ADVANCE_MODE = LB>
struct KernelPolicy {
    static constexpr int THREADS = _THREADS;
    static constexpr int ITEMS = _ITEMS_PER_THREAD;
    static constexpr int TILE = THREADS * ITEMS;
    static constexpr int MIN_BLOCKS = _MIN_BLOCKS_PER_CU;
    static constexpr int STAGE_CAPACITY = 2 * TILE;
    static constexpr MODE ADVANCE_MODE = _ADVANCE_MODE;
};

template <typename VertexId, typename SizeT>
struct AdvanceArgs {
    util::Frontier<VertexId, SizeT> in;
    util::Frontier<VertexId, SizeT> out;
    SizeT in_len;
    SizeT in_edges;
    const SizeT *d_row_offsets;
    const VertexId *d_column_indices;
    unsigned long long *d_tail_out;
    unsigned long long *d_tail_clear;
    int *d_overflow;
    BinPool<VertexId> bins;
    unsigned long long *d_duty = nullptr;
    const void *d_value_to_reduce = nullptr;
    void *d_reduced_value = nullptr;
};

template <bool FRESH, typename T>
__device__ __forceinline__ T LoadQueue(const T *p)
{
    if (FRESH) return __hip_atomic_load(p, __ATOMIC_RELAXED, __HIP_MEMORY_SCOPE_AGENT);
    return *p;
}

struct NoWriterStorage {};

struct NoReduce {
    static constexpr bool ENABLED = false;
};

template <REDUCE_OP OP, typename T>
struct ReduceOps {
    static_assert(OP != NONE && OP != MINUS && OP != MODULUS, "no neighbour-list reduction is defined for this REDUCE_OP");
    static __device__ __forceinline__ T Identity()
    {
        if (OP == MULTIPLIES) return static_cast<T>(1);
        if (OP == MAXIMUM) return std::numeric_limits<T>::lowest();
        if (OP == MINIMUM) return std::numeric_limits<T>::max();
        if (OP == BIT_AND) return static_cast<T>(~0ull);
        return static_cast<T>(0);
    }
    static __device__ __forceinline__ T Combine(T a, T b)
    {
        if constexpr (OP == MULTIPLIES) return a * b;
        else if constexpr (OP == MAXIMUM) return a > b ? a : b;
        else if constexpr (OP == MINIMUM) return a < b ? a : b;
        else if constexpr (OP == BIT_OR || OP == BIT_AND || OP == BIT_XOR) {
            static_assert(!(OP == BIT_OR || OP == BIT_AND || OP == BIT_XOR) || std::is_integral<T>::value, "bitwise reductions need an integer type");
            if constexpr (OP == BIT_OR) return a | b;
            else if constexpr (OP == BIT_AND) return a & b;
            else return a ^ b;
        } else return a + b;
    }
    static __device__ __forceinline__ void AtomicCombine(T *p, T v)
    {
        if constexpr (OP == PLUS && std::is_integral<T>::value && sizeof(T) == 8) {
            __hip_atomic_fetch_add(p, v, __ATOMIC_RELAXED, __HIP_MEMORY_SCOPE_AGENT);
        } else if constexpr (OP == PLUS) {
            atomicAdd(p, v);
        } else if constexpr (std::is_integral<T>::value && sizeof(T) == 8 && (OP == MAXIMUM || OP == MINIMUM)) {
            if constexpr (OP == MAXIMUM) __hip_atomic_fetch_max(p, v, __ATOMIC_RELAXED, __HIP_MEMORY_SCOPE_AGENT);
            else __hip_atomic_fetch_min(p, v, __ATOMIC_RELAXED, __HIP_MEMORY_SCOPE_AGENT);
        } else if constexpr (std::is_integral<T>::value && sizeof(T) == 4 && (OP == MAXIMUM || OP == MINIMUM || OP == BIT_OR || OP == BIT_AND || OP == BIT_XOR)) {
            if constexpr (OP == MAXIMUM) atomicMax(p, v);
            else if constexpr (OP == MINIMUM) atomicMin(p, v);
            else if constexpr (OP == BIT_OR) atomicOr(p, v);
            else if constexpr (OP == BIT_AND) atomicAnd(p, v);
            else atomicXor(p, v);
        } else {
            static_assert(sizeof(T) == 4, "32-bit values");
            unsigned *q = reinterpret_cast<unsigned *>(p);
            unsigned seen = __hip_atomic_load(q, __ATOMIC_RELAXED, __HIP_MEMORY_SCOPE_AGENT);
            for (;;) {
                T cur;
                __builtin_memcpy(&cur, &seen, 4);
                const T want = Combine(cur, v);
                unsigned bits;
                __builtin_memcpy(&bits, &want, 4);
                if (bits == seen) break;
                const unsigned old = atomicCAS(q, seen, bits);
                if (old == seen) break;
                seen = old;
            }
        }
    }
};

template <REDUCE_TYPE _R_TYPE, REDUCE_OP _R_OP, typename _Value, bool _BY_VERTEX = false>
struct Reduce {
    static constexpr bool ENABLED = true;
    static constexpr bool BY_VERTEX = _BY_VERTEX;
    static constexpr REDUCE_TYPE R_TYPE = _R_TYPE;
    static constexpr REDUCE_OP R_OP = _R_OP;
    typedef _Value Value;
    typedef ReduceOps<_R_OP, _Value> Ops;
};

template <typename KernelPolicy, typename VertexId, typename SizeT, bool WITH_WRITER = true>
// ... 42 lines not shown
    const int wave_base = __builtin_amdgcn_readfirstlane(tid / util::kWaveSize) * (util::kWaveSize * ITEMS);
    const long long total = a.in_edges;

    SizeT cursor = 0;
    if (tile_begin > 0) {
        const SizeT first_slot = static_cast<SizeT>(tile_begin * TILE);
        SizeT lo = 0, hi = a.in_len;
        while (hi - lo > 1) {
            const SizeT step = (hi - lo + util::kWaveSize - 1) / util::kWaveSize;
            const long long idx = static_cast<long long>(lo) + static_cast<long long>(lane) * step;
            const bool le = idx < hi && LoadQueue<FRESH>(a.in.scan + idx) <= first_slot;
            const int last = __popcll(__ballot(le)) - 1;
            const long long next_hi = static_cast<long long>(lo) + static_cast<long long>(last + 1) * step;
            lo = static_cast<SizeT>(lo + static_cast<long long>(last) * step);
            if (next_hi < hi) hi = static_cast<SizeT>(next_hi);
        }
        cursor = lo;
    }

    const long long slot_end = (tile_end * TILE < total) ? tile_end * TILE : total;
    long long slot_at = tile_begin * TILE;
    SizeT p_scan = INT_MAX, p_row = 0;
    VertexId p_v = 0;
    constexpr bool STAGED = HasSourceData<Functor, VertexId, typename ProblemData::DataSlice>::value;
    typedef typename EdgeStateOf<Functor, STAGED>::type EdgeState;
    unsigned p_source = 0u;
    if (slot_at < slot_end && cursor + tid < a.in_len) {
        p_scan = LoadQueue<FRESH>(a.in.scan + cursor + tid);
        p_row = LoadQueue<FRESH>(a.in.row_start + cursor + tid);
        p_v = LoadQueue<FRESH>(a.in.v + cursor + tid);
        if constexpr (STAGED) p_source = Functor::SourceData(p_v, &slice);
    }

    while (slot_at < slot_end) {
        const SizeT slot0 = static_cast<SizeT>(slot_at);
        const int limit = (slot_end - slot_at < TILE) ? static_cast<int>(slot_end - slot_at) : TILE;
        if (++tile_tag > MAX_TAG) {
            __syncthreads();
#pragma unroll
            for (int k = 0; k < ITEMS; ++k) sh.own[k * THREADS + tid] = 0u;
            tile_tag = 1u;
            __syncthreads();
        }
        const unsigned tag = tile_tag << IDX_BITS;

        int pending = 0;
        if constexpr (!COUNT_ONLY) pending = Writer::Count(sh.writer);

        {
            const SizeT rel = (p_scan == INT_MAX) ? INT_MAX : p_scan - slot0;
            sh.scan[tid] = rel;
            if (rel < limit) {
                sh.row[tid] = p_row;
                sh.vertex[tid] = p_v;
                if constexpr (STAGED) sh.source_data[tid] = p_source;
                if (rel > 0) sh.own[rel] = tag | static_cast<unsigned>(tid);
            }
            const unsigned long long in_tile = __ballot(rel < limit);
            if (lane == 0) sh.owner_count[tile_tag & 1][tid / util::kWaveSize] = __popcll(in_tile);
        }
        if (FRESH) __syncthreads();
        else util::LdsBarrier();
        int owners = 0;
#pragma unroll
        for (int w = 0; w < THREADS / util::kWaveSize; ++w) owners += sh.owner_count[tile_tag & 1][w];
        int slots = limit;
        if (owners == THREADS) {
            slots = sh.scan[THREADS - 1];
            owners = THREADS - 1;
        }
        int advance = owners - 1;
        if (sh.scan[owners] == slots) advance = owners;
        {
            const SizeT idx = cursor + advance + tid;
            p_scan = INT_MAX;
            if (slot_at + slots < slot_end && idx < a.in_len) {
                p_scan = LoadQueue<FRESH>(a.in.scan + idx);
                p_row = LoadQueue<FRESH>(a.in.row_start + idx);
                p_v = LoadQueue<FRESH>(a.in.v + idx);
            }
        }
        if constexpr (!COUNT_ONLY) {
            if (pending > KernelPolicy::STAGE_CAPACITY - TILE) {
                if (OUT_WITH_DEGREES) Writer::template Flush<true>(sh.writer, pending, a.out, a.d_tail_out, a.d_overflow, a.d_row_offsets);
                else Writer::FlushIds(sh.writer, pending, a.out.v, a.out.capacity, a.d_tail_out, a.d_overflow);
            }
        }

        SizeT edge[ITEMS];
        VertexId src[ITEMS];
        VertexId dst[ITEMS];
        bool live[ITEMS];
        int own[Reducer::ENABLED ? ITEMS : 1];
        unsigned source[STAGED ? ITEMS : 1];
        EdgeState state[STAGED ? ITEMS : 1];
        {
            int lo = 0, hi = owners;
            if (wave_base > 0) {
                while (hi - lo > 1) {
                    const int mid = (lo + hi) >> 1;
                    if (sh.scan[mid] <= wave_base) lo = mid; else hi = mid;
                }
            }
            unsigned carry = tag | static_cast<unsigned>(lo);
#pragma unroll
            for (int k = 0; k < ITEMS; ++k) {
                const int slot = wave_base + k * util::kWaveSize + static_cast<int>(lane);
                live[k] = slot < slots;
                unsigned m = sh.own[slot];
                if (lane == 0) m = max(m, carry);
                m = util::WaveInclusiveMaxDpp(m);
                carry = static_cast<unsigned>(__builtin_amdgcn_readlane(static_cast<int>(m), util::kWaveSize - 1));
                const int owner = static_cast<int>(m & static_cast<unsigned>(THREADS - 1));
                edge[k] = sh.row[owner] + (slot - sh.scan[owner]);
                src[k] = sh.vertex[owner];
                if constexpr (STAGED) source[k] = sh.source_data[owner];
                if constexpr (Reducer::ENABLED) own[k] = owner;
            }
        }
#pragma unroll
        for (int k = 0; k < ITEMS; ++k) {
            if (!live[k]) { edge[k] = 0; src[k] = 0; }
            dst[k] = a.d_column_indices[edge[k]];
        }
#pragma unroll
        for (int k = 0; k < ITEMS; ++k) {
            bool pass;
            if constexpr (STAGED)
                pass = Functor::ScreenEdge(src[k], dst[k], &slice, edge[k], slot0 + wave_base + k * util::kWaveSize + static_cast<int>(lane),
                                           source[k], state[k]);
            else
                pass = ScreenEdge<Functor>(src[k], dst[k], &slice, edge[k], slot0 + wave_base + k * util::kWaveSize + static_cast<int>(lane));
            live[k] = live[k] & pass;
        }
        if constexpr (STAGED) {
            p_source = 0u;
            if (p_scan != INT_MAX) p_source = Functor::SourceData(p_v, &slice);
        }
        int mine = 0;
        if constexpr (BINNED) {
            static_assert(!BINNED || COUNT_ONLY, "a binned advance enqueues nothing itself");
            Binner<THREADS, ITEMS, VertexId, ProblemData::MARK_PREDECESSORS>::Put(sh.binner, a.bins, src, dst, live);
#pragma unroll
            for (int k = 0; k < ITEMS; ++k) mine += live[k] ? 1 : 0;
        } else {
            if constexpr (STAGED) {
                typedef decltype(Functor::IssueEdge(src[0], dst[0], &slice, edge[0], slot0, source[0], state[0])) Token;
                Token token[ITEMS];
#pragma unroll
                for (int k = 0; k < ITEMS; ++k) {
                    token[k] = Token();
                    if (live[k]) token[k] = Functor::IssueEdge(src[k], dst[k], &slice, edge[k],
                                                               slot0 + wave_base + k * util::kWaveSize + static_cast<int>(lane), source[k], state[k]);
                }
#pragma unroll
                for (int k = 0; k < ITEMS; ++k)
                    live[k] = live[k] && Functor::ResolveEdge(token[k], src[k], dst[k], &slice, edge[k],
                                                              slot0 + wave_base + k * util::kWaveSize + static_cast<int>(lane), state[k]);
            } else if constexpr (HasIssueEdge<Functor, VertexId, typename ProblemData::DataSlice>::value) {
                typedef decltype(Functor::IssueEdge(src[0], dst[0], &slice, edge[0], slot0)) Token;
                Token token[ITEMS];
#pragma unroll
                for (int k = 0; k < ITEMS; ++k) {
                    token[k] = Token();
                    if (live[k]) token[k] = Functor::IssueEdge(src[k], dst[k], &slice, edge[k],
                                                               slot0 + wave_base + k * util::kWaveSize + static_cast<int>(lane));
                }
// ... 252 lines not shown
                        TYPE  = V2V)
{
    if (args.in_len <= 0 || args.in_edges <= 0) return hipSuccess;
    const long long tiles = (static_cast<long long>(args.in_edges) + KernelPolicy::TILE - 1) / KernelPolicy::TILE;
    if (max_grid_size <= 0)
        max_grid_size = util::ResidentGrid(LoadBalancedKernel<KernelPolicy, ProblemData, Functor, OUT_WITH_DEGREES, COUNT_ONLY>, KernelPolicy::THREADS);
    long long grid = tiles < max_grid_size ? tiles : max_grid_size;
    if (grid < 1) grid = 1;
    hipLaunchKernelGGL((LoadBalancedKernel<KernelPolicy, ProblemData, Functor, OUT_WITH_DEGREES, COUNT_ONLY>), dim3(static_cast<unsigned>(grid)),
                       dim3(KernelPolicy::THREADS), 0, stream, args, slice);
    return util::GRError("advance::LoadBalancedKernel launch failed", __FILE__, __LINE__);
}

template <typename KernelPolicy, typename ProblemData, typename Functor, typename Reducer>
__global__ __launch_bounds__(KernelPolicy::THREADS) void ReduceKernel(
    AdvanceArgs<typename ProblemData::VertexId, typename ProblemData::SizeT> a, typename ProblemData::DataSlice slice)
{
    typedef typename ProblemData::VertexId VertexId;
    typedef typename ProblemData::SizeT SizeT;
    typedef AdvanceShared<KernelPolicy, VertexId, SizeT, false> Shared;
    __shared__ Shared sh;
    unsigned tile_tag;
    InitOwnerMarks<KernelPolicy>(sh, tile_tag);
    const long long tiles = (static_cast<long long>(a.in_edges) + KernelPolicy::TILE - 1) / KernelPolicy::TILE;
    const long long per_block = (tiles + gridDim.x - 1) / gridDim.x;
    const long long tile_begin = static_cast<long long>(blockIdx.x) * per_block;
    const long long tile_end = (tile_begin + per_block < tiles) ? tile_begin + per_block : tiles;
    if (tile_begin >= tile_end) return;
    __syncthreads();
    unsigned accepted = 0;
    ExpandTiles<KernelPolicy, ProblemData, Functor, false, false, true, false, Reducer>(a, slice, tile_begin, tile_end, sh, accepted, tile_tag);
}

template <typename T>
__global__ void FillKernel(T *d_out, T value, long long n)
{
    const long long stride = static_cast<long long>(gridDim.x) * blockDim.x;
    for (long long i = static_cast<long long>(blockIdx.x) * blockDim.x + threadIdx.x; i < n; i += stride) d_out[i] = value;
}

template <REDUCE_OP OP, typename T>
inline T HostIdentity()
{
    if (OP == MULTIPLIES) return static_cast<T>(1);
    if (OP == MAXIMUM) return std::numeric_limits<T>::lowest();
    if (OP == MINIMUM) return std::numeric_limits<T>::max();
    if (OP == BIT_AND) return static_cast<T>(~0ull);
    return static_cast<T>(0);
}

template <typename KernelPolicy, typename ProblemData, typename Functor, REDUCE_TYPE R_TYPE, REDUCE_OP R_OP, typename Value, bool BY_VERTEX = false>
hipError_t LaunchReduce(AdvanceArgs<typename ProblemData::VertexId, typename ProblemData::SizeT> args,
                        const typename ProblemData::DataSlice &slice, const Value *d_value_to_reduce, Value *d_reduced_value,
                        int max_grid_size, hipStream_t stream, long long out_len = 0, bool prefill = true)
{
    static_assert(R_TYPE != EMPTY && R_OP != NONE, "a reducing advance needs a reduction");
    static_assert(R_OP != MINUS && R_OP != MODULUS, "MINUS and MODULUS are not associative: no neighbour-list reduction is defined for them");
    if (out_len <= 0) out_len = args.in_len;
    if (out_len <= 0) return hipSuccess;
    hipError_t rc = hipSuccess;
    if (prefill) {
        hipLaunchKernelGGL((FillKernel<Value>), dim3(static_cast<unsigned>((out_len + 1023) / 1024 < 2048 ? (out_len + 1023) / 1024 : 2048)),
                           dim3(256), 0, stream, d_reduced_value, HostIdentity<R_OP, Value>(), out_len);
        rc = util::GRError("advance::FillKernel launch failed", __FILE__, __LINE__);
    }
    if (rc || args.in_edges <= 0 || args.in_len <= 0) return rc;
    args.d_value_to_reduce = d_value_to_reduce;
    args.d_reduced_value = d_reduced_value;
    typedef Reduce<R_TYPE, R_OP, Value, BY_VERTEX> Reducer;
    const long long tiles = (static_cast<long long>(args.in_edges) + KernelPolicy::TILE - 1) / KernelPolicy::TILE;
    if (max_grid_size <= 0) max_grid_size = util::ResidentGrid(ReduceKernel<KernelPolicy, ProblemData, Functor, Reducer>, KernelPolicy::THREADS);
    long long grid = tiles < max_grid_size ? tiles : max_grid_size;
    if (grid < 1) grid = 1;
    hipLaunchKernelGGL((ReduceKernel<KernelPolicy, ProblemData, Functor, Reducer>), dim3(static_cast<unsigned>(grid)),
                       dim3(KernelPolicy::THREADS), 0, stream, args, slice);
    return util::GRError("advance::ReduceKernel launch failed", __FILE__, __LINE__);
}

struct GridBarrierState {
    unsigned *d_counter;
    int *d_timeout;
};

__device__ __forceinline__ bool GridBarrier(const GridBarrierState &b, unsigned &epoch)
{
    __shared__ int s_ok;
    asm volatile("s_waitcnt vmcnt(0)" ::: "memory");
    __syncthreads();
    if (threadIdx.x == 0) {
        __builtin_amdgcn_fence(__ATOMIC_RELEASE, "agent");
        asm volatile("s_waitcnt vmcnt(0)" ::: "memory");
        epoch += 1;
        const unsigned target = epoch * gridDim.x;
        __hip_atomic_fetch_add(b.d_counter, 1u, __ATOMIC_RELAXED, __HIP_MEMORY_SCOPE_AGENT);
        int ok = 1;
        unsigned spins = 0;
        while (__hip_atomic_load(b.d_counter, __ATOMIC_RELAXED, __HIP_MEMORY_SCOPE_AGENT) < target) {
            __builtin_amdgcn_s_sleep(2);
            if (++spins > 4000000u || __hip_atomic_load(b.d_timeout, __ATOMIC_RELAXED, __HIP_MEMORY_SCOPE_AGENT)) {
                __hip_atomic_store(b.d_timeout, 1, __ATOMIC_RELAXED, __HIP_MEMORY_SCOPE_AGENT);
                ok = 0;
                break;
            }
        }
        __builtin_amdgcn_fence(__ATOMIC_ACQUIRE, "agent");
        asm volatile("s_waitcnt vmcnt(0)" ::: "memory");
        if (__hip_atomic_load(b.d_timeout, __ATOMIC_RELAXED, __HIP_MEMORY_SCOPE_AGENT)) ok = 0;
        s_ok = ok;
    }
    __syncthreads();
    return s_ok != 0;
}

template <typename VertexId, typename SizeT>
struct PersistentArgs {
    TailArgs<VertexId, SizeT> t;
    GridBarrierState barrier;
    SizeT solo_edges;
    long long unexplored_edges;
    double switch_factor;
    SizeT leave_below = 0;
};

template <typename KernelPolicy, typename ProblemData, typename Functor>
__device__ __forceinline__ void PersistentLevelsBody(const PersistentArgs<typename ProblemData::VertexId, typename ProblemData::SizeT> &p,
                                                     typename ProblemData::DataSlice &slice, const long long first_iteration)
{
    typedef typename ProblemData::VertexId VertexId;
    typedef typename ProblemData::SizeT SizeT;
    typedef AdvanceShared<KernelPolicy, VertexId, SizeT> Shared;
    typedef typename Shared::Writer Writer;
    __shared__ Shared sh;
    const TailArgs<VertexId, SizeT> &t = p.t;

    Writer::Init(sh.writer);
    unsigned tile_tag;
    InitOwnerMarks<KernelPolicy>(sh, tile_tag);
    int selector = t.selector;
    long long iteration = first_iteration;
    long long unexplored = p.unexplored_edges;
    int done = 0;
    unsigned epoch = 0;
    bool solo = (gridDim.x == 1);
    unsigned long long sum_len = 0, sum_edges = 0;
    for (;;) {
        if (threadIdx.x == 0) {
            sh.level_tail = __hip_atomic_load(t.d_tail + (iteration & 3), __ATOMIC_RELAXED, __HIP_MEMORY_SCOPE_AGENT);
            if (blockIdx.x == 0)
                __hip_atomic_store(t.d_tail + ((iteration + 2) & 3), 0ull, __ATOMIC_RELAXED, __HIP_MEMORY_SCOPE_AGENT);
        }
        __syncthreads();
        const unsigned long long tail = sh.level_tail;
        const SizeT len = static_cast<SizeT>(util::TailCount(tail));
        const SizeT edges = static_cast<SizeT>(util::TailEdges(tail));
        if (len == 0 || edges > t.edge_limit || done >= t.max_levels) break;
        if (p.switch_factor > 0 && static_cast<double>(edges) * p.switch_factor > static_cast<double>(unexplored)) break;
        if (p.leave_below > 0 && done > 0 && edges < p.leave_below) break;
        if (!solo && edges <= p.solo_edges) {
            if (blockIdx.x != 0) return;
            solo = true;
        } else if (solo && gridDim.x > 1 && edges > p.solo_edges)
            break;

        AdvanceArgs<VertexId, SizeT> a;
        a.in = t.queue[selector];
        a.out = t.queue[selector ^ 1];
        a.in_len = len;
        a.in_edges = edges;
        a.d_row_offsets = t.d_row_offsets;
        a.d_column_indices = t.d_column_indices;
        a.d_tail_out = t.d_tail + ((iteration + 1) & 3);
        a.d_tail_clear = nullptr;
        a.d_overflow = t.d_overflow;
        slice.iteration = static_cast<VertexId>(iteration);

        const long long tiles = (static_cast<long long>(edges) + KernelPolicy::TILE - 1) / KernelPolicy::TILE;
        const long long per_block = solo ? tiles : (tiles + gridDim.x - 1) / gridDim.x;
        const long long tile_begin = static_cast<long long>(blockIdx.x) * per_block;
        const long long tile_end = (tile_begin + per_block < tiles) ? tile_begin + per_block : tiles;
        if (tile_begin < tile_end) {
            unsigned accepted = 0;
            ExpandTiles<KernelPolicy, ProblemData, Functor, true, true>(a, slice, tile_begin, tile_end, sh, accepted, tile_tag);
            const int rest = Writer::Count(sh.writer);
            __syncthreads();
            Writer::template Flush<true>(sh.writer, rest, a.out, a.d_tail_out, a.d_overflow, a.d_row_offsets);
        }
        if (solo) {
            asm volatile("s_waitcnt vmcnt(0)" ::: "memory");
            __syncthreads();
        } else if (!GridBarrier(p.barrier, epoch))
            break;
        selector ^= 1;
        ++iteration;
        ++done;
        sum_len += len;
        sum_edges += edges;
        unexplored -= edges;
    }
    if (blockIdx.x == 0 && threadIdx.x == 0) {
        *t.d_levels_done = done;
        t.d_level_sums[0] = sum_len;
        t.d_level_sums[1] = sum_edges;
    }
}

template <typename KernelPolicy, typename ProblemData, typename Functor>
__global__ __launch_bounds__(KernelPolicy::THREADS) void PersistentLevelsKernel(
    PersistentArgs<typename ProblemData::VertexId, typename ProblemData::SizeT> p, typename ProblemData::DataSlice slice)
{
    PersistentLevelsBody<KernelPolicy, ProblemData, Functor>(p, slice, p.t.first_iteration);
}

template <typename KernelPolicy, typename ProblemData, typename Functor>
__global__ __launch_bounds__(KernelPolicy::THREADS) void ChainedPersistentLevelsKernel(
    PersistentArgs<typename ProblemData::VertexId, typename ProblemData::SizeT> p, typename ProblemData::DataSlice slice,
    SweepChain chain, int sweeps, long long first_level, const int *d_queue_invalid, int *d_gate)
{
    const ChainEnd end = ChainOutcome(chain, sweeps, util::LaneId());
    const bool run = end.action == kSweepSwitch && end.end >= 2 && end.prev_action == kSweepSparseEmit && *d_queue_invalid == 0;
    if (blockIdx.x == 0 && threadIdx.x == 0) {
        d_gate[0] = run ? 1 : 0;
        d_gate[1] = end.end - 1;
        if (!run) {
            *p.t.d_levels_done = 0;
            p.t.d_level_sums[0] = 0ull;
            p.t.d_level_sums[1] = 0ull;
        }
    }
    if (!run) return;
    PersistentLevelsBody<KernelPolicy, ProblemData, Functor>(p, slice, first_level + (end.end - 1));
}

template <typename KernelPolicy, typename ProblemData, typename Functor>
hipError_t LaunchPersistentLevels(const PersistentArgs<typename ProblemData::VertexId, typename ProblemData::SizeT> &args,
                                  const typename ProblemData::DataSlice &slice, int cu_count, int grid_hint, hipStream_t stream,
                                  bool cooperative = false)
{
    int grid = util::ResidentGrid(PersistentLevelsKernel<KernelPolicy, ProblemData, Functor>, KernelPolicy::THREADS);
    if (grid > cu_count) grid = cu_count;
    if (grid_hint > 0 && grid_hint < grid) grid = grid_hint;
    if (grid < 1) grid = 1;
    if (cooperative) {
        PersistentArgs<typename ProblemData::VertexId, typename ProblemData::SizeT> a = args;
        typename ProblemData::DataSlice s = slice;
        void *params[] = {&a, &s};
        return util::GRError(hipLaunchCooperativeKernel(reinterpret_cast<const void *>(&PersistentLevelsKernel<KernelPolicy, ProblemData, Functor>),
                                                        dim3(grid), dim3(KernelPolicy::THREADS), params, 0, stream),
                             "advance::PersistentLevelsKernel cooperative launch failed", __FILE__, __LINE__);
    }
    hipLaunchKernelGGL((PersistentLevelsKernel<KernelPolicy, ProblemData, Functor>), dim3(grid), dim3(KernelPolicy::THREADS), 0,
                       stream, args, slice);
    return util::GRError("advance::PersistentLevelsKernel launch failed", __FILE__, __LINE__);
}

template <typename KernelPolicy, typename ProblemData, typename Functor>
hipError_t LaunchChainedPersistentLevels(const PersistentArgs<typename ProblemData::VertexId, typename ProblemData::SizeT> &args,
                                         const typename ProblemData::DataSlice &slice, int cu_count, const SweepChain &chain, int sweeps,
                                         long long first_level, const int *d_queue_invalid, int *d_gate, hipStream_t stream)
{
    int grid = util::ResidentGrid(ChainedPersistentLevelsKernel<KernelPolicy, ProblemData, Functor>, KernelPolicy::THREADS);
    if (grid > cu_count) grid = cu_count;
    if (grid < 1) grid = 1;
    hipLaunchKernelGGL((ChainedPersistentLevelsKernel<KernelPolicy, ProblemData, Functor>), dim3(grid), dim3(KernelPolicy::THREADS), 0, stream, args,
                       slice, chain, sweeps, first_level, d_queue_invalid, d_gate);
    return util::GRError("advance::ChainedPersistentLevelsKernel launch failed", __FILE__, __LINE__);
}

template <typename KernelPolicy, typename ProblemData, typename Functor>
hipError_t LaunchTailLevels(const TailArgs<typename ProblemData::VertexId, typename ProblemData::SizeT> &args,
                            const typename ProblemData::DataSlice &slice, hipStream_t stream)
{
    hipLaunchKernelGGL((TailLevelsKernel<KernelPolicy, ProblemData, Functor>), dim3(1), dim3(KernelPolicy::THREADS), 0, stream,
                       args, slice);
    return util::GRError("advance::TailLevelsKernel launch failed", __FILE__, __LINE__);
}

}
}
}
```

gunrockinst_amd/csrc/gunrock/oprtr/frontier_writer.hpp:

```cpp
#pragma once

#include <hip/hip_runtime.h>

#include <gunrock/util/device_intrinsics.hpp>
#include <gunrock/util/frontier.hpp>

namespace gunrock {
namespace oprtr {

template <int THREADS, int CAPACITY, typename VertexId, typename SizeT>
struct FrontierWriter {
    static_assert(CAPACITY % THREADS == 0, "staging capacity must be a multiple of the workgroup size");
    static constexpr int PER_THREAD = CAPACITY / THREADS;
    typedef util::BlockScan<THREADS, unsigned long long> Scan;

    struct Storage {
        VertexId buf[CAPACITY];
        typename Scan::Storage scan;
        unsigned long long base;
        int count;
    };

    static __device__ __forceinline__ void Init(Storage &st)
    {
        if (threadIdx.x == 0) st.count = 0;
    }

    static __device__ __forceinline__ void Append(Storage &st, bool pred, VertexId v)
    {
        const unsigned long long m = __ballot(pred);
        if (m == 0) return;
        const int leader = __ffsll(static_cast<long long>(m)) - 1;
        int base = 0;
        if (static_cast<int>(util::LaneId()) == leader) base = atomicAdd(&st.count, __popcll(m));
        base = __shfl(base, leader, util::kWaveSize);
        if (pred) st.buf[base + util::RankInMask(m)] = v;
    }

    static __device__ __forceinline__ int Reserve(Storage &st, int mine)
    {
        const int incl = util::WaveInclusiveSum(mine);
        const int total = __shfl(incl, util::kWaveSize - 1, util::kWaveSize);
        int base = 0;
        if (total == 0) return 0;
        if (util::LaneId() == util::kWaveSize - 1) base = atomicAdd(&st.count, total);
        base = __shfl(base, util::kWaveSize - 1, util::kWaveSize);
        return base + incl - mine;
    }

    static __device__ __forceinline__ int Count(const Storage &st) { return st.count; }

    template <bool DROP_ZERO_DEGREE>
    static __device__ __forceinline__ void Flush(Storage &st, const int n,
                                                 const util::Frontier<VertexId, SizeT> &out,
                                                 unsigned long long *d_tail, int *d_overflow,
                                                 const SizeT *__restrict__ d_row_offsets)
    {
        if (n == 0) return;

        VertexId v[PER_THREAD];
        SizeT rs[PER_THREAD];
        SizeT deg[PER_THREAD];
        unsigned long long mine = 0;
#pragma unroll
        for (int j = 0; j < PER_THREAD; ++j) {
            const int i = j * THREADS + threadIdx.x;
            deg[j] = -1;
            if (i < n) {
                v[j] = st.buf[i];
                rs[j] = d_row_offsets[v[j]];
                deg[j] = d_row_offsets[v[j] + 1] - rs[j];
                if (DROP_ZERO_DEGREE && deg[j] == 0) deg[j] = -1;
                if (deg[j] >= 0) mine += util::PackTail(1u, static_cast<unsigned>(deg[j]));
            }
        }
        unsigned long long total;
        const unsigned long long excl = Scan::ExclusiveSum(mine, total, st.scan);
        if (threadIdx.x == 0) {
            st.base = total ? atomicAdd(d_tail, total) : 0ull;
            st.count = 0;
        }
        __syncthreads();
        const unsigned long long block_base = st.base;
        if (static_cast<unsigned long long>(util::TailCount(block_base)) + util::TailCount(total) >
            static_cast<unsigned long long>(out.capacity)) {
            if (threadIdx.x == 0) *d_overflow = 1;
            return;
        }
        unsigned pos = util::TailCount(block_base) + util::TailCount(excl);
        unsigned epos = util::TailEdges(block_base) + util::TailEdges(excl);
#pragma unroll
        for (int j = 0; j < PER_THREAD; ++j) {
            if (deg[j] >= 0) {
                out.v[pos] = v[j];
                out.row_start[pos] = rs[j];
                out.scan[pos] = static_cast<SizeT>(epos);
                ++pos;
                epos += static_cast<unsigned>(deg[j]);
            }
        }
    }

    static __device__ __forceinline__ void FlushIds(Storage &st, const int n, VertexId *d_out, SizeT capacity,
                                                    unsigned long long *d_tail, int *d_overflow)
    {
        if (n == 0) return;
        if (threadIdx.x == 0) {
            st.base = atomicAdd(d_tail, static_cast<unsigned long long>(n));
            st.count = 0;
        }
        VertexId v[PER_THREAD];
#pragma unroll
        for (int j = 0; j < PER_THREAD; ++j) {
            const int i = j * THREADS + threadIdx.x;
            if (i < n) v[j] = st.buf[i];
        }
        __syncthreads();
        const unsigned long long base = util::TailCount(st.base);
        if (base + static_cast<unsigned long long>(n) > static_cast<unsigned long long>(capacity)) {
            if (threadIdx.x == 0) *d_overflow = 1;
            return;
        }
#pragma unroll
        for (int j = 0; j < PER_THREAD; ++j) {
            const int i = j * THREADS + threadIdx.x;
            if (i < n) d_out[base + i] = v[j];
        }
        __syncthreads();
    }
};

}
}
```

gunrockinst_amd/csrc/lib/bfs_app.hip:

```cpp
#include <gunrock/gunrock.h>
#include <gunrock/gunrock_mi355x.h>

#include <cstdio>
#include <cstdlib>

#include <gunrock/app/bfs/bfs_enactor.hpp>
#include <gunrock/app/bfs/bfs_problem.hpp>
#include <gunrock/app/handle_runner.hpp>
#include <gunrock/graphio/device_sort.hpp>
#include <gunrock/graphio/symmetry.hpp>
#include <gunrock/oprtr/filter/kernel.hpp>
#include <gunrock/csr.hpp>
#include <gunrock/graphio/utils.hpp>
#include <gunrock/util/context.hpp>

using namespace gunrock;
using namespace gunrock::app;
using namespace gunrock::app::bfs;

namespace {

struct BfsRunner {
    virtual ~BfsRunner() {}
    virtual hipError_t Init(const Csr<int, int, int> &g) = 0;
    virtual hipError_t InitDevice(int nodes, int edges, int *d_ro, int *d_ci) = 0;
    virtual hipError_t SetInverse(const int *d_iro, const int *d_ici, float alpha, float beta) = 0;
    virtual hipError_t AutoInverse(bool &enabled, bool &built, float &build_ms, bool build_if_directed = true) = 0;
    virtual void SetTuning(float alpha, float beta, float lite_factor, int tail_edge_limit) = 0;
    virtual void SetPersistentLimit(int limit) = 0;
    virtual void SetTwcLimit(int limit) = 0;
    virtual void SetCooperativeLaunch(bool on) = 0;
    virtual void SetBinnedMinEdges(long long min_edges) = 0;
    virtual void SetLabelDeferral(int enabled, int mask_limit) = 0;
    virtual int SetOption(const char *name, double value) = 0;
    virtual void SetHeadPass(int min_edges, int max_edges) = 0;
    virtual hipError_t Reset(int src, double queue_sizing) = 0;
    virtual hipError_t Enact(int src, int max_grid_size, int traversal_mode, float *ms) = 0;
    virtual void Stats(long long &queued, long long &depth, double &duty, long long &launches, double &kernel_ms) = 0;
    virtual int Trace(int max_levels, long long *frontier, long long *edges, double *ms, int *kind) = 0;
    virtual hipError_t Extract(int *labels, int *preds) = 0;
    virtual void DeviceResults(int **labels, int **preds) = 0;
    virtual void BuildRelabelled(bool on) = 0;
    virtual long long MaskFlushes() = 0;
    virtual void RelabelInfo(long long &hubs, long long &with_edges, int &threshold, float &build_ms, long long &bytes) = 0;
};

template <bool PRED, bool IDEMP, bool INSTR>
struct BfsRunnerT : BfsRunner {
    typedef BFSProblem<int, int, int, PRED, IDEMP, (PRED && IDEMP)> Problem;
    util::DeviceContext context;
    Problem problem;
    BFSEnactor<INSTR> enactor;
    EventPair timer;

    explicit BfsRunnerT(int device) : context(device), enactor(false) { timer.Create(); }
    ~BfsRunnerT() override { FreeInverse(); }
    hipError_t Init(const Csr<int, int, int> &g) override { return problem.Init(false, g, 1); }
    hipError_t InitDevice(int nodes, int edges, int *d_ro, int *d_ci) override
    {
        return problem.InitFromDevice(nodes, edges, d_ro, d_ci);
    }
    hipError_t SetInverse(const int *d_iro, const int *d_ici, float alpha, float beta) override
    {
        if (!problem.data_slices) return hipErrorNotInitialized;
        if (!d_iro || !d_ici) return problem.InverseIsSelf(alpha, beta);
        return problem.SetInverseGraph(d_iro, d_ici, alpha, beta);
    }
    hipError_t AutoInverse(bool &enabled, bool &built, float &build_ms, bool build_if_directed) override
    {
        hipError_t retval = hipSuccess;
        enabled = false;
        built = false;
        build_ms = 0.f;
        if (!problem.data_slices || problem.nodes <= 0 || problem.edges <= 0) return retval;
        GraphSlice<int, int, int> *gs = problem.graph_slices[0];
        bool symmetric = false;
        GR_CHECK(graphio::DeviceIsSymmetric(problem.nodes, problem.edges, gs->d_row_offsets, gs->d_column_indices, gs->stream, symmetric),
                 "BFS symmetry check failed");
        if (symmetric) {
            GR_CHECK(problem.InverseIsSelf(), "BFS InverseIsSelf failed");
            enabled = true;
            return retval;
        }
        if (!build_if_directed) return retval;
        if ((retval = timer.Timed(gs->stream, &build_ms, [&]() { return BuildInverse(gs); }))) return retval;
        enabled = true;
        built = true;
        return retval;
    }
    hipError_t BuildInverse(GraphSlice<int, int, int> *gs)
    {
        hipError_t retval = hipSuccess;
        FreeInverse();
        GR_CHECK(hipMalloc(&d_inv_row_offsets, sizeof(int) * (static_cast<size_t>(problem.nodes) + 1)), "BFS hipMalloc inverse offsets failed");
        GR_CHECK(hipMalloc(&d_inv_column_indices, sizeof(int) * static_cast<size_t>(problem.edges)), "BFS hipMalloc inverse columns failed");
        GR_CHECK(graphio::DeviceTransposeCsr(problem.nodes, problem.edges, gs->d_row_offsets, gs->d_column_indices, d_inv_row_offsets,
                                             d_inv_column_indices, gs->stream),
                 "BFS transpose failed");
        GR_CHECK(problem.SetInverseGraph(d_inv_row_offsets, d_inv_column_indices), "BFS SetInverseGraph failed");
        return retval;
    }
    void FreeInverse()
    {
        if (d_inv_row_offsets) util::GRError(hipFree(d_inv_row_offsets), "BFS hipFree inverse offsets failed", __FILE__, __LINE__);
        if (d_inv_column_indices) util::GRError(hipFree(d_inv_column_indices), "BFS hipFree inverse columns failed", __FILE__, __LINE__);
        d_inv_row_offsets = nullptr;
        d_inv_column_indices = nullptr;
    }
    int *d_inv_row_offsets = nullptr;
    int *d_inv_column_indices = nullptr;
    void SetPersistentLimit(int limit) override { problem.persistent_edge_limit = limit; }
    void SetTwcLimit(int limit) override { problem.twc_edge_limit = limit; }
    void SetCooperativeLaunch(bool on) override { problem.cooperative_launch = on; }
    void SetBinnedMinEdges(long long min_edges) override { problem.binned_min_edges = min_edges; }
    int SetOption(const char *name, double value) override
    {
        const std::string key(name ? name : "");
        if (key == "emit_queue_factor") problem.emit_queue_factor = static_cast<float>(value);
        else if (key == "sparse_sweep_div") problem.sparse_sweep_div = static_cast<int>(value);
        else if (key == "speculative_emit") problem.speculative_emit = value != 0.0;
        else if (key == "chain_sweeps") problem.chain_sweeps = static_cast<int>(value);
        else if (key == "chain_closing") problem.chain_closing = value != 0.0;
        else if (key == "label_pass") problem.label_pass = value != 0.0 ? 1 : 0;
        else if (key == "walk_queue") problem.walk_queue = value != 0.0 ? 1 : 0;
        else if (key == "relabel") {
            if (value > 0.0 && !problem.HasRelabelled()) return 2;
            problem.relabel = value > 0.0 ? 1 : (value < 0.0 ? -1 : 0);
        } else if (key == "relabel_min_nodes") {
            if (value < 0.0) return 2;
            problem.relabel_min_nodes = static_cast<long long>(value);
        } else if (key == "relabel_hubs") {
            if (value < 0.0) return 2;
            const long long hubs = static_cast<long long>(value);
            if (!problem.HasRelabelled()) problem.relabel_hubs = hubs;
            else if (hubs != problem.relabel_hubs && problem.BuildRelabelled(hubs) != hipSuccess) return 3;
        } else return 1;
        return 0;
    }
    void BuildRelabelled(bool on) override { problem.build_relabelled = on; }
    long long MaskFlushes() override { return problem.mask_flushes; }
    void RelabelInfo(long long &hubs, long long &with_edges, int &threshold, float &build_ms, long long &bytes) override
    {
        const bool ready = problem.HasRelabelled();
        hubs = ready ? problem.relabelled.hubs : -1;
        with_edges = ready ? problem.relabelled.with_edges : -1;
        threshold = ready ? problem.relabelled.threshold : 0;
        build_ms = ready ? problem.relabelled.build_ms : 0.f;
        const long long n = problem.nodes, words = (n + 63) / 64 + 2;
        bytes = ready ? static_cast<long long>(problem.relabelled.bytes) + words * 8 + (words + 1) * 4 + n * 8 + n * 4 * (problem.MARK_PREDECESSORS ? 2 : 1) : 0;
    }
    void SetLabelDeferral(int enabled, int mask_limit) override
    {
        if (enabled >= 0) problem.defer_labels = enabled != 0;
        if (mask_limit > 0) problem.level_mask_limit = mask_limit;
    }
    void SetHeadPass(int min_edges, int max_edges) override
    {
        problem.head_pass_min_edges = min_edges;
        problem.head_pass_max_edges = max_edges;
    }
    void SetTuning(float alpha, float beta, float lite_factor, int tail_edge_limit) override
    {
        if (alpha > 0) problem.alpha = alpha;
        if (beta > 0) problem.beta = beta;
        if (lite_factor >= 0) problem.lite_factor = lite_factor;
        if (tail_edge_limit >= 0) problem.tail_edge_limit = tail_edge_limit;
    }
    hipError_t Reset(int src, double queue_sizing) override
    {
        return problem.Reset(src, enactor.GetFrontierType(), queue_sizing);
    }
    hipError_t Enact(int src, int max_grid_size, int traversal_mode, float *ms) override
    {
        return timer.Timed(problem.graph_slices[0]->stream, ms, [&]() { return enactor.template Enact<Problem>(context, &problem, src, max_grid_size, traversal_mode); });
    }
    void Stats(long long &queued, long long &depth, double &duty, long long &launches, double &kernel_ms) override
    {
        enactor.GetStatistics(queued, depth, duty);
        enactor.GetKernelStatistics(launches, kernel_ms);
    }
    int Trace(int max_levels, long long *frontier, long long *edges, double *ms, int *kind) override
    {
        const auto &t = enactor.GetLevelTrace();
        return CopyTrace(t.size(), max_levels, Column(frontier, [&](int i) { return t[i].frontier; }), Column(edges, [&](int i) { return t[i].edges; }),
                         Column(ms, [&](int i) { return t[i].ms; }), Column(kind, [&](int i) { return t[i].kind; }));
    }
    hipError_t Extract(int *labels, int *preds) override { return problem.Extract(labels, preds); }
    void DeviceResults(int **labels, int **preds) override
    {
        if (labels) *labels = problem.data_slices ? problem.d_out_labels : nullptr;
        if (preds) *preds = problem.data_slices ? problem.d_out_preds : nullptr;
    }
};

BfsRunner *MakeRunner(bool pred, bool idemp, bool instr, int device)
{
    if (instr) {
        if (pred) return idemp ? static_cast<BfsRunner *>(new BfsRunnerT<true, true, true>(device))
                               : new BfsRunnerT<true, false, true>(device);
        return idemp ? static_cast<BfsRunner *>(new BfsRunnerT<false, true, true>(device))
                     : new BfsRunnerT<false, false, true>(device);
    }
    if (pred) return idemp ? static_cast<BfsRunner *>(new BfsRunnerT<true, true, false>(device))
                           : new BfsRunnerT<true, false, false>(device);
    return idemp ? static_cast<BfsRunner *>(new BfsRunnerT<false, true, false>(device))
                 : new BfsRunnerT<false, false, false>(device);
}

void DisplayStats(const char *name, int src, const int *h_labels, const Csr<int, int, int> &graph, double elapsed,
                  long long search_depth, long long total_queued, double avg_duty)
{
    long long nodes_visited = 0, edges_visited = 0;
    grx_bfs_count_visited(graph.nodes, graph.row_offsets, h_labels, &nodes_visited, &edges_visited);
    double redundant_work = 0.0;
    if (total_queued > 0 && edges_visited > 0)
        redundant_work = 100.0 * (static_cast<double>(total_queued) - edges_visited) / edges_visited;
    std::printf("[%s] finished.", name);
    if (nodes_visited < 5) {
        std::printf("Fewer than 5 vertices visited.\n");
        return;
    }
    const double m_teps = static_cast<double>(edges_visited) / (elapsed * 1000.0);
    std::printf("\nelapsed: %.3f ms, rate: %.3f MiEdges/s", elapsed, m_teps);
// ... 82 lines not shown
    p->runner->SetBinnedMinEdges(min_edges);
    return 0;
}

int grx_bfs_set_cooperative_launch(grx_bfs *p, int on)
{
    if (!p || !p->runner) return 1;
    p->runner->SetCooperativeLaunch(on != 0);
    return 0;
}

int grx_bfs_set_persistent_limit(grx_bfs *p, int edge_limit)
{
    if (!p || !p->runner || edge_limit < 0) return 1;
    p->runner->SetPersistentLimit(edge_limit);
    return 0;
}

int grx_bfs_set_twc_limit(grx_bfs *p, int edge_limit)
{
    if (!p || !p->runner || edge_limit < 0) return 1;
    p->runner->SetTwcLimit(edge_limit);
    return 0;
}

int grx_bfs_set_tuning(grx_bfs *p, float alpha, float beta, float lite_factor, int tail_edge_limit)
{
    if (!p) return -1;
    p->runner->SetTuning(alpha, beta, lite_factor, tail_edge_limit);
    return 0;
}

int grx_bfs_reset(grx_bfs *p, int src, double queue_sizing)
{
    if (!p) return -1;
    return static_cast<int>(p->runner->Reset(src, queue_sizing));
}

int grx_bfs_enact(grx_bfs *p, int src, int max_grid_size, int traversal_mode, float *elapsed_ms)
{
    if (!p) return -1;
    return static_cast<int>(p->runner->Enact(src, max_grid_size, traversal_mode, elapsed_ms));
}

int grx_bfs_stats(grx_bfs *p, long long *total_queued, long long *search_depth, double *avg_duty,
                  long long *kernel_launches, double *kernel_ms)
{
    if (!p) return -1;
    long long q = 0, d = 0, l = 0;
    double duty = 0, kms = 0;
    p->runner->Stats(q, d, duty, l, kms);
    if (total_queued) *total_queued = q;
    if (search_depth) *search_depth = d;
    if (avg_duty) *avg_duty = duty;
    if (kernel_launches) *kernel_launches = l;
    if (kernel_ms) *kernel_ms = kms;
    return 0;
}

int grx_bfs_level_trace(grx_bfs *p, int max_levels, long long *frontier, long long *edges, double *ms, int *kind)
{
    if (!p || max_levels < 0) return -1;
    return p->runner->Trace(max_levels, frontier, edges, ms, kind);
}

int grx_bfs_extract(grx_bfs *p, int *h_labels, int *h_preds)
{
    if (!p || !h_labels) return -1;
    return static_cast<int>(p->runner->Extract(h_labels, h_preds));
}

int grx_bfs_device_results(grx_bfs *p, int **d_labels, int **d_preds)
{
    if (!p) return -1;
    p->runner->DeviceResults(d_labels, d_preds);
    return 0;
}

int grx_bfs_mask_flushes(grx_bfs *p, long long *flushes)
{
    if (!p || !p->runner || !flushes) return -1;
    *flushes = p->runner->MaskFlushes();
    return 0;
}

int grx_bfs_relabel_info(grx_bfs *p, long long *hubs, long long *with_edges, int *threshold, float *build_ms, long long *bytes)
{
    if (!p || !p->runner) return -1;
    long long h = -1, we = -1, b = 0;
    int t = 0;
    float ms = 0.f;
    p->runner->RelabelInfo(h, we, t, ms, b);
    if (hubs) *hubs = h;
    if (with_edges) *with_edges = we;
    if (threshold) *threshold = t;
    if (build_ms) *build_ms = ms;
    if (bytes) *bytes = b;
    return 0;
}

int grx_filter_queue(int n, const int *d_in, const int *d_row_offsets, int capacity, int *d_out_v, int *d_out_row_start, int *d_out_scan,
                     int *out_len, long long *out_edges, int max_grid_size)
{
    typedef BFSProblem<int, int, int, false, false, false> Problem;
    typedef BFSFunctor<int, int, int, Problem> Functor;
    typedef oprtr::filter::KernelPolicy<256, 4, 8> Policy;
    if (n < 0 || !d_out_v || !out_len || (d_row_offsets && (!d_out_row_start || !d_out_scan))) return -1;
    hipError_t retval = hipSuccess;
    unsigned long long *d_tail = nullptr;
    int *d_overflow = nullptr;
    GR_CHECK(hipMalloc(&d_tail, sizeof(unsigned long long)), "grx_filter_queue hipMalloc failed");
    GR_CHECK(hipMalloc(&d_overflow, sizeof(int)), "grx_filter_queue hipMalloc failed");
    GR_CHECK(hipMemset(d_tail, 0, sizeof(unsigned long long)), "grx_filter_queue memset failed");
    GR_CHECK(hipMemset(d_overflow, 0, sizeof(int)), "grx_filter_queue memset failed");
    GR_CHECK(hipDeviceSynchronize(), "grx_filter_queue sync failed");
    oprtr::filter::FilterArgs<int, int> f;
    f.d_in = d_in;
    f.num_elements = n;
    f.out.v = d_out_v;
    f.out.row_start = d_out_row_start;
    f.out.scan = d_out_scan;
    f.out.capacity = capacity;
    f.d_tail_out = d_tail;
    f.d_tail_clear = nullptr;
    f.d_overflow = d_overflow;
    f.d_row_offsets = d_row_offsets;
    Problem::DataSlice slice{};
    const int grid = max_grid_size > 0 ? max_grid_size : 2048;
    if (n > 0) {
        if (d_row_offsets) retval = oprtr::filter::LaunchKernel<Policy, Problem, Functor, true>(f, slice, grid, 0);
        else retval = oprtr::filter::LaunchKernel<Policy, Problem, Functor, false>(f, slice, grid, 0);
    }
    unsigned long long tail = 0;
    int overflow = 0;
    if (!retval) retval = util::GRError(hipMemcpy(&tail, d_tail, sizeof(tail), hipMemcpyDeviceToHost), "grx_filter_queue read failed", __FILE__, __LINE__);
    if (!retval) retval = util::GRError(hipMemcpy(&overflow, d_overflow, sizeof(int), hipMemcpyDeviceToHost), "grx_filter_queue read failed", __FILE__, __LINE__);
    hipFree(d_tail);
    hipFree(d_overflow);
    if (retval) return static_cast<int>(retval);
    if (overflow) return static_cast<int>(util::GRError(hipErrorInvalidConfiguration, "Frontier queue overflow. Please increase queue-sizing factor.", __FILE__, __LINE__));
    *out_len = static_cast<int>(util::TailCount(tail));
    if (out_edges) *out_edges = static_cast<long long>(util::TailEdges(tail));
    return 0;
}

void grx_bfs_destroy(grx_bfs *p)
{
    if (!p) return;
    delete p->runner;
    delete p;
}

void gunrock_bfs_func(struct GunrockGraph *graph_out, const struct GunrockGraph *graph_in, struct GunrockConfig configs,
                      struct GunrockDataType data_type)
{
    if (!graph_out || !graph_in) return;
    if (data_type.VTXID_TYPE != VTXID_INT || data_type.SIZET_TYPE != SIZET_INT) return;
    if (data_type.VALUE_TYPE != VALUE_INT) {
        std::printf("Not Yet Support This DataType Combination.\n");
        return;
    }
    BorrowedCsr<> borrowed(static_cast<int>(graph_in->num_nodes), static_cast<int>(graph_in->num_edges), static_cast<int *>(graph_in->row_offsets),
                           static_cast<int *>(graph_in->col_indices));
    Csr<int, int, int> &csr = borrowed.graph;

    int src = 0;
// ... 34 lines not shown
```

include/gunrock/gunrock_mi355x.h:

```cpp
#ifndef GUNROCK_GUNROCK_MI355X_H_
#define GUNROCK_GUNROCK_MI355X_H_

#include <stddef.h>
#include <stdint.h>

#ifdef __cplusplus
extern "C" {
#endif

typedef struct grx_graph grx_graph;

int grx_graph_from_market(const char *path, int undirected, int reversed, grx_graph **out);
int grx_graph_from_market_cached(const char *path, int undirected, int reversed, int *cache_hit, grx_graph **out);
int grx_graph_rmat_libc(int nodes, int edges, int undirected, double a, double b, double c, double d, grx_graph **out);
int grx_graph_rmat_seeded(int scale, long long pairs, uint64_t seed, int undirected,
                          double a, double b, double c, double d, grx_graph **out);
int grx_graph_from_coo(int nodes, long long tuples, const int *rows, const int *cols, const int *vals, grx_graph **out);
int grx_graph_from_csr(int nodes, int edges, const int *row_offsets, const int *col_indices, const int *edge_values,
                       grx_graph **out);
int grx_graph_nodes(const grx_graph *g);
int grx_graph_edges(const grx_graph *g);
const int *grx_graph_row_offsets(const grx_graph *g);
const int *grx_graph_col_indices(const grx_graph *g);
const int *grx_graph_edge_values(const grx_graph *g);
int grx_graph_highest_degree_node(grx_graph *g, int *max_degree);
int grx_graph_average_degree(grx_graph *g);
int grx_random_node(int num_nodes);
void grx_graph_free(grx_graph *g);

int grx_rmat_seeded_device(int scale, long long first, long long count, uint64_t seed,
                           double a, double b, double c, double d, int *d_rows, int *d_cols, void *stream);

typedef struct grx_coo2csr grx_coo2csr;
int grx_coo_to_csr_sort(grx_coo2csr **handle, int rows, int nodes, long long pairs, const int *d_rows, const int *d_cols,
                        int undirected, int parts, int rank, long long *edges_out, void *stream);
int grx_coo_to_csr_emit(grx_coo2csr *handle, int *d_row_offsets, int *d_col_indices, void *stream);
void grx_coo_to_csr_free(grx_coo2csr *handle);

typedef struct grx_bfs grx_bfs;

int grx_bfs_create(grx_bfs **out, int mark_pred, int idempotence, int instrument, int device);
int grx_bfs_init(grx_bfs *p, int nodes, int edges, const int *row_offsets, const int *col_indices);
int grx_bfs_init_device(grx_bfs *p, int nodes, int edges, int *d_row_offsets, int *d_col_indices);
int grx_bfs_set_inverse_graph(grx_bfs *p, const int *d_inv_row_offsets, const int *d_inv_col_indices,
                              float alpha, float beta);
int grx_bfs_auto_inverse(grx_bfs *p, int build_if_directed, int *enabled, int *built, float *build_ms);
int grx_bfs_set_tuning(grx_bfs *p, float alpha, float beta, float lite_factor, int tail_edge_limit);
int grx_bfs_set_persistent_limit(grx_bfs *p, int edge_limit);
int grx_bfs_set_twc_limit(grx_bfs *p, int edge_limit);
int grx_bfs_set_cooperative_launch(grx_bfs *p, int on);
int grx_bfs_set_binned_min_edges(grx_bfs *p, long long min_edges);
int grx_bfs_set_label_deferral(grx_bfs *p, int enabled, int mask_limit);
int grx_bfs_set_option(grx_bfs *p, const char *name, double value);
int grx_bfs_mask_flushes(grx_bfs *p, long long *flushes);
int grx_bfs_relabel_info(grx_bfs *p, long long *hubs, long long *with_edges, int *threshold, float *build_ms, long long *bytes);
int grx_bfs_set_head_pass(grx_bfs *p, int min_edges, int max_edges);
int grx_bfs_reset(grx_bfs *p, int src, double queue_sizing);
int grx_bfs_enact(grx_bfs *p, int src, int max_grid_size, int traversal_mode, float *elapsed_ms);
int grx_bfs_stats(grx_bfs *p, long long *total_queued, long long *search_depth, double *avg_duty,
                  long long *kernel_launches, double *kernel_ms);
int grx_bfs_level_trace(grx_bfs *p, int max_levels, long long *frontier, long long *edges, double *ms, int *kind);
int grx_bfs_extract(grx_bfs *p, int *h_labels, int *h_preds);
int grx_bfs_device_results(grx_bfs *p, int **d_labels, int **d_preds);
void grx_bfs_destroy(grx_bfs *p);
int grx_filter_queue(int n, const int *d_in, const int *d_row_offsets, int capacity, int *d_out_v, int *d_out_row_start, int *d_out_scan,
                     int *out_len, long long *out_edges, int max_grid_size);

enum grx_advance_mode { GRX_ADVANCE_IDS = 0, GRX_ADVANCE_FRONTIER = 1, GRX_ADVANCE_COUNT_ONLY = 2 };
enum grx_advance_rule { GRX_ADVANCE_RULE_MASK = 0, GRX_ADVANCE_RULE_CLAIM = 1 };
enum grx_advance_functor { GRX_ADVANCE_FUNCTOR_PLAIN = 0, GRX_ADVANCE_FUNCTOR_HOOKED = 1 };
enum grx_reduce_type { GRX_REDUCE_VERTEX = 1, GRX_REDUCE_EDGE = 2 };
enum grx_reduce_op {
    GRX_REDUCE_PLUS = 1, GRX_REDUCE_MINUS = 2, GRX_REDUCE_MULTIPLIES = 3, GRX_REDUCE_MODULUS = 4, GRX_REDUCE_BIT_OR = 5,
    GRX_REDUCE_BIT_AND = 6, GRX_REDUCE_BIT_XOR = 7, GRX_REDUCE_MAXIMUM = 8, GRX_REDUCE_MINIMUM = 9
};
enum grx_value_type { GRX_VALUE_INT = 0, GRX_VALUE_UINT = 1, GRX_VALUE_FLOAT = 2, GRX_VALUE_LONGLONG = 3, GRX_VALUE_ULONGLONG = 4 };
int grx_advance_queue(const int *d_row_offsets, const int *d_col_indices, const int *d_in_v, const int *d_in_row_start,
                      const int *d_in_scan, int in_len, int in_edges, int mode, int rule, int functor, const int *d_mask, int *d_labels,
                      int depth, int *d_edge_hits, int *d_edge_src, int capacity, int *d_out_v, int *d_out_row_start, int *d_out_scan,
                      int *out_len, long long *out_edges, int max_grid_size);
int grx_advance_reduce(const int *d_row_offsets, const int *d_col_indices, const int *d_in_v, const int *d_in_row_start,
                       const int *d_in_scan, int in_len, int in_edges, int r_type, int r_op, int value_type, int by_vertex, int prefill,
                       long long out_len, const void *d_values, void *d_reduced, int functor, const int *d_mask, int *d_edge_hits,
                       int *d_edge_src, int max_grid_size);

void grx_bfs_count_visited(int nodes, const int *row_offsets, const int *labels,
                           long long *nodes_visited, long long *edges_visited);

typedef struct grx_cc grx_cc;

int grx_cc_create(grx_cc **out, int instrument, int device);
int grx_cc_init(grx_cc *p, int nodes, int edges, const int *row_offsets, const int *col_indices);
int grx_cc_init_device(grx_cc *p, int nodes, int edges, int *d_row_offsets, int *d_col_indices);
int grx_cc_reset(grx_cc *p);
int grx_cc_enact(grx_cc *p, int max_grid_size, float *elapsed_ms);
int grx_cc_stats(grx_cc *p, long long *edge_sweeps, long long *vertex_sweeps, long long *kernel_launches, double *kernel_ms);
int grx_cc_mirrored(grx_cc *p, int *mirrored);
int grx_cc_sweep_edges(grx_cc *p, long long *edges);
int grx_cc_extract(grx_cc *p, int *h_component_ids, unsigned *num_components);
int grx_cc_device_results(grx_cc *p, int **d_component_ids);
void grx_cc_destroy(grx_cc *p);

typedef struct grx_mst grx_mst;

int grx_mst_create(grx_mst **out, int instrument, int device);
int grx_mst_init(grx_mst *p, int nodes, int edges, const int *row_offsets, const int *col_indices, const int *edge_values);
int grx_mst_init_device(grx_mst *p, int nodes, int edges, int *d_row_offsets, int *d_col_indices, int *d_edge_values);
int grx_mst_reset(grx_mst *p);
int grx_mst_enact(grx_mst *p, int max_grid_size, float *elapsed_ms);
int grx_mst_stats(grx_mst *p, long long *rounds, long long *edges_scanned, long long *kernel_launches, double *kernel_ms);
int grx_mst_round_trace(grx_mst *p, int max_rounds, long long *entries, double *ms);
int grx_mst_extract(grx_mst *p, int *h_selected , long long *total_weight, int *forest_edges);
int grx_mst_device_results(grx_mst *p, int **d_selected);
void grx_mst_destroy(grx_mst *p);

typedef struct grx_mis grx_mis;
enum { GRX_MIS_SET = 0, GRX_MIS_COLOR_ROUNDS = 1, GRX_MIS_COLOR_FIRST_FIT = 2 };

int grx_mis_create(grx_mis **out, int instrument, int device);
int grx_mis_init(grx_mis *p, int nodes, int edges, const int *row_offsets, const int *col_indices, const int *priorities,
                 unsigned seed);
int grx_mis_init_device(grx_mis *p, int nodes, int edges, int *d_row_offsets, int *d_col_indices, int *d_priorities, unsigned seed);
int grx_mis_set_tail(grx_mis *p, int enable);
int grx_mis_reset(grx_mis *p);
int grx_mis_enact(grx_mis *p, int mode, int max_grid_size, float *elapsed_ms);
int grx_mis_stats(grx_mis *p, long long *rounds, long long *tail_sweeps, long long *entries_read, long long *polls,
                  long long *kernel_launches, double *kernel_ms);
int grx_mis_round_trace(grx_mis *p, int max_rounds, long long *vertices, double *ms);
int grx_mis_extract(grx_mis *p, int *h_ids , long long *summary);
int grx_mis_device_results(grx_mis *p, int **d_ids);
void grx_mis_destroy(grx_mis *p);

typedef struct grx_tc grx_tc;
enum { GRX_TC_AUTO = 0, GRX_TC_LANE = 1, GRX_TC_LDS = 2, GRX_TC_GLOBAL = 3 };

int grx_tc_create(grx_tc **out, int instrument, int device);
int grx_tc_init(grx_tc *p, int nodes, int edges, const int *row_offsets, const int *col_indices);
// ... 125 lines not shown
```

Before: 1.017 million MTEPS.

## Fuse closing chained persistent levels with tiled label emission in one kernel

When label deferral is on and the closing chain qualifies, a fused variant of the chained persistent levels kernel runs. It reserves a subset of workgroups to emit tiled labels while the rest finish the closing levels, and logs vertices discovered during the closing phase so their labels can be patched afterwards. This aims to remove the separate gated label-emission launch and overlap label writing with the tail traversal. In exchange it adds a discovery log with an overflow fallback, cross-workgroup arrival counters and extra shared memory, which may lower occupancy or slow the closing levels.

```diff
diff --git a/gunrockinst_amd/capi.py b/gunrockinst_amd/capi.py
--- a/gunrockinst_amd/capi.py
+++ b/gunrockinst_amd/capi.py
@@ -103,6 +103,7 @@
     "grx_bfs_extract": (C.c_int, [C.c_void_p, i32p, i32p]),
     "grx_bfs_device_results": (C.c_int, [C.c_void_p, C.POINTER(C.c_void_p), C.POINTER(C.c_void_p)]),
     "grx_bfs_mask_flushes": (C.c_int, [C.c_void_p, C.POINTER(C.c_longlong)]),
+    "grx_bfs_closing_info": (C.c_int, [C.c_void_p, C.POINTER(C.c_longlong), C.POINTER(C.c_longlong), C.POINTER(C.c_longlong)]),
     "grx_bfs_relabel_info": (C.c_int, [C.c_void_p, C.POINTER(C.c_longlong), C.POINTER(C.c_longlong), C.POINTER(C.c_int),
                                        C.POINTER(C.c_float), C.POINTER(C.c_longlong)]),
     "grx_bfs_destroy": (None, [C.c_void_p]),
@@ -503,6 +504,11 @@
         _check(lib().grx_bfs_mask_flushes(self._h, C.byref(v)), "grx_bfs_mask_flushes")
         return v.value
 
+    def closing_info(self):
+        f, v, o = C.c_longlong(), C.c_longlong(), C.c_longlong()
+        _check(lib().grx_bfs_closing_info(self._h, C.byref(f), C.byref(v), C.byref(o)), "grx_bfs_closing_info")
+        return {"fused_launches": f.value, "patched_vertices": v.value, "log_overflows": o.value}
+
     def relabel_info(self):
         h, we, t, ms, b = C.c_longlong(), C.c_longlong(), C.c_int(), C.c_float(), C.c_longlong()
         _check(lib().grx_bfs_relabel_info(self._h, C.byref(h), C.byref(we), C.byref(t), C.byref(ms), C.byref(b)),
diff --git a/gunrockinst_amd/csrc/gunrock/app/bfs/bfs_enactor.hpp b/gunrockinst_amd/csrc/gunrock/app/bfs/bfs_enactor.hpp
--- a/gunrockinst_amd/csrc/gunrock/app/bfs/bfs_enactor.hpp
+++ b/gunrockinst_amd/csrc/gunrock/app/bfs/bfs_enactor.hpp
@@ -328,7 +328,7 @@
             if (queued == 0) return util::GRError(hipErrorInvalidValue, "BFSEnactor: no frontier bitmap for a bottom-up sweep", __FILE__, __LINE__);
             const bool closing_queued = problem->chain_closing && problem->persistent_edge_limit > 0;
             int *d_gate = work_progress.d_chain_log + 8;
-            bool emit_queued = false;
+            bool emit_queued = false, fused = false;
             if (closing_queued) {
                 oprtr::advance::PersistentArgs<VertexId, SizeT> p;
                 p.t.queue[0] = gs->frontier_queues[0];
@@ -356,10 +356,38 @@
                 chain.index = queued;
                 chain.first_may_switch = 0;
                 chain.d_log = work_progress.d_chain_log;
-                if ((rc = oprtr::advance::LaunchChainedPersistentLevels<PersistentPolicy, BFSProblem, BfsFunctor>(
+                if (deferring && problem->ClosingFusable(queued)) {
+                    if ((rc = problem->EnsureClosingLog())) return rc;
+                    VertexId labels[oprtr::advance::kChainMax];
+                    for (int k = 1; k <= queued; ++k) labels[k - 1] = static_cast<VertexId>(it0 + k);
+                    oprtr::advance::ClosingFuse fuse;
+                    fuse.log.d_entries = problem->d_closing_log;
+                    fuse.log.d_count = problem->d_closing_words;
+                    fuse.log.capacity = problem->closing_log_capacity;
+                    fuse.d_arrived = problem->d_closing_words + 1;
+                    fuse.d_log_overflow = work_progress.d_chain_log;
+                    fuse.d_counters = problem->d_closing_counters;
+                    const int *d_invalid = reinterpret_cast<const int *>(work_progress.AuxTail());
+                    if (problem->active == 1) {
+                        typedef TiledLabelRole<VertexId, true, BFSProblem::MARK_PREDECESSORS> Role;
+                        typename Role::Args la;
+                        problem->template FillLabelRole<true, BFSProblem::MARK_PREDECESSORS>(la, masks + 1, labels, queued);
+                        rc = oprtr::advance::LaunchChainedClosingFused<PersistentPolicy, BFSProblem, BfsFunctor, Role>(
+                            p, *ds, cu_count, chain, queued, it0, d_invalid, d_gate, la, fuse, stream, fused, problem->closing_workgroups);
+                    } else {
+                        typedef TiledLabelRole<VertexId, false, false> Role;
+                        typename Role::Args la;
+                        problem->template FillLabelRole<false, false>(la, masks + 1, labels, queued);
+                        rc = oprtr::advance::LaunchChainedClosingFused<PersistentPolicy, BFSProblem, BfsFunctor, Role>(
+                            p, *ds, cu_count, chain, queued, it0, d_invalid, d_gate, la, fuse, stream, fused, problem->closing_workgroups);
+                    }
+                    if (rc) return rc;
+                    emit_queued = fused;
+                }
+                if (!fused && (rc = oprtr::advance::LaunchChainedPersistentLevels<PersistentPolicy, BFSProblem, BfsFunctor>(
                          p, *ds, cu_count, chain, queued, it0, reinterpret_cast<const int *>(work_progress.AuxTail()), d_gate, stream)))
                     return rc;
-                if (deferring && problem->speculative_emit && problem->level_masks.count + queued <= app::bfs::kLevelMasks) {
+                if (!fused && deferring && problem->speculative_emit && problem->level_masks.count + queued <= app::bfs::kLevelMasks) {
                     VertexId labels[oprtr::advance::kChainMax];
                     for (int k = 1; k <= queued; ++k) labels[k - 1] = static_cast<VertexId>(it0 + k);
                     if ((rc = problem->EmitLabelsGated(stream, masks + 1, labels, queued, d_gate))) return rc;
@@ -413,7 +441,8 @@
                 queue_emitted = false;
                 out_slot_clean = false;
                 snapshot_valid = false;
-                if (emit_queued) problem->emit_current = queue_length == 0;
+                if (emit_queued) problem->emit_current = queue_length == 0 && !(fused && work_progress.box->chain_log[0] != 0);
+                if (fused) ++problem->closing_fused_launches;
             }
             return rc;
         };
diff --git a/gunrockinst_amd/csrc/gunrock/app/bfs/bfs_problem.hpp b/gunrockinst_amd/csrc/gunrock/app/bfs/bfs_problem.hpp
--- a/gunrockinst_amd/csrc/gunrock/app/bfs/bfs_problem.hpp
+++ b/gunrockinst_amd/csrc/gunrock/app/bfs/bfs_problem.hpp
@@ -292,90 +292,123 @@
         e[p] |= spread[row | (__builtin_amdgcn_alignbit(hi[p], lo[p], x) & 0xFu)];
 }
 
+struct TiledLabelsShared {
+    LabelPlanes planes[2][2 * kLabelSpan];
+    uint2 s_tier[2][2 * kLabelTileWords];
+    int table[16];
+    unsigned char spread[256];
+};
+
+template <bool RELABEL>
+__device__ __forceinline__ void TiledLabelsRuns(const graphio::RelabelView &map, long long w0, long long &xw1, long long &xwh)
+{
+    xw1 = w0;
+    xwh = 0;
+    if (RELABEL) {
+        xw1 = (map.hubs + map.d_base1[w0]) >> 6;
+        if (map.hubs > 0) xwh = map.d_base0[w0] >> 6;
+    }
+}
+
+
+struct TiledLabelsLoads {
+    unsigned long long m[kLevelMasks], vis, nev, tile_edge, tile_hub;
+    unsigned tile_base1, tile_base0;
+    bool live;
+};
+
+template <typename VertexId, bool RELABEL>
+__device__ __forceinline__ void TiledLabelsLoad(TiledLabelsLoads &r, const LevelMaskList<VertexId> &levels, const unsigned long long *d_visited,
+                                                const unsigned long long *d_never, const graphio::RelabelView &map, const long long nodes,
+                                                const int t, const long long w0, const long long xw1, const long long xwh)
+{
+    const long long words = (nodes + 63) / 64;
+    const bool hubs = RELABEL && map.hubs > 0;
+    r.tile_edge = r.tile_hub = 0ull;
+    r.tile_base1 = r.tile_base0 = 0u;
+    if (RELABEL && t < kLabelTileWords && w0 + t < words) {
+        r.tile_edge = map.d_edge[w0 + t];
+        r.tile_base1 = map.d_base1[w0 + t];
+        if (hubs) {
+            r.tile_hub = map.d_hub[w0 + t];
+            r.tile_base0 = map.d_base0[w0 + t];
+        }
+    }
+    const int tier = t >> 7, col = t & 127;
+    r.live = false;
+    r.vis = r.nev = 0ull;
+#pragma unroll
+    for (int k = 0; k < kLevelMasks; ++k) r.m[k] = 0ull;
+    if (col < kLabelSpan && (tier == 0 || hubs)) {
+        const long long word = (tier ? xwh : xw1) + col;
+        r.live = col < (RELABEL ? kLabelTileWords + 1 : kLabelTileWords) && word < words;
+        const long long at = r.live ? word : 0;
+#pragma unroll
+        for (int k = 0; k < kLevelMasks; ++k) r.m[k] = levels.mask[k][at];
+        r.vis = d_visited[at];
+        r.nev = (!RELABEL && d_never) ? d_never[at] : 0ull;
+    }
+}
+
+template <typename VertexId, bool RELABEL>
+__device__ __forceinline__ void TiledLabelsFold(const TiledLabelsLoads &r, const LevelMaskList<VertexId> &levels, const graphio::RelabelView &map,
+                                                TiledLabelsShared &lds, const int t, const int valid)
+{
+    const bool hubs = RELABEL && map.hubs > 0;
+    if (t < 16) lds.table[t] = (t >= 1 && t <= kLevelMasks) ? levels.label[t - 1] : -1;
+    if (RELABEL) {
+        unsigned dealt = 0u;
+        for (int b = 0, q = 0; b < 4; ++b)
+            if ((t >> (4 + b)) & 1) {
+                dealt |= ((static_cast<unsigned>(t) >> q) & 1u) << b;
+                ++q;
+            }
+        lds.spread[t] = static_cast<unsigned char>(dealt);
+    }
+    const int tier = t >> 7, col = t & 127;
+    if (col < kLabelSpan && (tier == 0 || hubs)) {
+        unsigned long long pl[4] = {0ull, 0ull, 0ull, 0ull}, later = 0ull;
+#pragma unroll
+        for (int k = kLevelMasks - 1; k >= 0; --k) {
+            const unsigned long long own = (k < valid ? r.m[k] : 0ull) & ~later;
+            later |= own;
+#pragma unroll
+            for (int p = 0; p < 4; ++p)
+                if (((k + 1) >> p) & 1) pl[p] |= own;
+        }
+        const unsigned long long kept = r.vis & ~r.nev & ~later;
+#pragma unroll
+        for (int p = 0; p < 4; ++p) {
+            if ((kCodeWorkLabel >> p) & 1u) pl[p] |= kept;
+            if (!r.live) pl[p] = 0ull;
+        }
+        lds.planes[tier][2 * col] = LabelPlanes{static_cast<unsigned>(pl[0]), static_cast<unsigned>(pl[1]), static_cast<unsigned>(pl[2]), static_cast<unsigned>(pl[3])};
+        lds.planes[tier][2 * col + 1] = LabelPlanes{static_cast<unsigned>(pl[0] >> 32), static_cast<unsigned>(pl[1] >> 32), static_cast<unsigned>(pl[2] >> 32),
+                                                    static_cast<unsigned>(pl[3] >> 32)};
+    }
+    if (RELABEL && t < kLabelTileWords) {
+        const unsigned e_lo = static_cast<unsigned>(r.tile_edge), h_lo = static_cast<unsigned>(r.tile_hub);
+        const unsigned x1 = static_cast<unsigned>(map.hubs) + r.tile_base1;
+        lds.s_tier[0][2 * t] = make_uint2(e_lo, x1);
+        lds.s_tier[0][2 * t + 1] = make_uint2(static_cast<unsigned>(r.tile_edge >> 32), x1 + __popc(e_lo));
+        lds.s_tier[1][2 * t] = make_uint2(h_lo, r.tile_base0);
+        lds.s_tier[1][2 * t + 1] = make_uint2(static_cast<unsigned>(r.tile_hub >> 32), r.tile_base0 + __popc(h_lo));
+    }
+}
+
 template <typename VertexId, bool RELABEL, bool PRED>
-__global__ __launch_bounds__(256) void TiledLabelsKernel(LevelMaskList<VertexId> levels, const unsigned long long *d_visited,
-                                                         const unsigned long long *d_never, graphio::RelabelView map, long long nodes,
-                                                         VertexId src, const VertexId *d_work_labels, const VertexId *d_work_preds,
-                                                         const VertexId *d_old_of_new, VertexId *d_labels, VertexId *d_preds)
+__device__ __forceinline__ void TiledLabelsStore(const graphio::RelabelView &map, const long long nodes, const VertexId src,
+                                                 const VertexId *d_work_labels, const VertexId *d_work_preds, const VertexId *d_old_of_new,
+                                                 VertexId *d_labels, VertexId *d_preds, const TiledLabelsShared &lds, const int t, const long long w0,
+                                                 const long long xw1, const long long xwh)
 {
     typedef __attribute__((ext_vector_type(4))) int V4;
-    __shared__ LabelPlanes planes[2][2 * kLabelSpan];
-    __shared__ uint2 s_tier[2][2 * kLabelTileWords];
-    __shared__ int table[16];
-    __shared__ unsigned char spread[256];
-    const int t = threadIdx.x;
+    const LabelPlanes (&planes)[2][2 * kLabelSpan] = lds.planes;
+    const uint2 (&s_tier)[2][2 * kLabelTileWords] = lds.s_tier;
+    const int (&table)[16] = lds.table;
+    const unsigned char (&spread)[256] = lds.spread;
     const long long words = (nodes + 63) / 64;
-    const long long w0 = static_cast<long long>(blockIdx.x) * kLabelTileWords;
     const bool hubs = RELABEL && map.hubs > 0;
-    long long xw1 = w0, xwh = 0;
-    if (RELABEL) {
-        xw1 = (map.hubs + map.d_base1[w0]) >> 6;
-        if (hubs) xwh = map.d_base0[w0] >> 6;
-    }
-    int valid = levels.count;
-    if (levels.d_gate) {
-        const int go = levels.d_gate[0], filled = levels.d_gate[1];
-        if (go == 0) return;
-        valid = levels.chain_first + filled;
-    }
-    if (t < 16) table[t] = (t >= 1 && t <= kLevelMasks) ? levels.label[t - 1] : -1;
-    if (RELABEL) {
-        unsigned dealt = 0u;
-        for (int b = 0, r = 0; b < 4; ++b)
-            if ((t >> (4 + b)) & 1) {
-                dealt |= ((static_cast<unsigned>(t) >> r) & 1u) << b;
-                ++r;
-            }
-        spread[t] = static_cast<unsigned char>(dealt);
-    }
-    unsigned long long tile_edge = 0ull, tile_hub = 0ull;
-    unsigned tile_base1 = 0u, tile_base0 = 0u;
-    if (RELABEL && t < kLabelTileWords && w0 + t < words) {
-        tile_edge = map.d_edge[w0 + t];
-        tile_base1 = map.d_base1[w0 + t];
-        if (hubs) {
-            tile_hub = map.d_hub[w0 + t];
-            tile_base0 = map.d_base0[w0 + t];
-        }
-    }
-    const int tier = t >> 7, col = t & 127;
-    if (col < kLabelSpan && (tier == 0 || hubs)) {
-        const long long word = (tier ? xwh : xw1) + col;
-        const bool live = col < (RELABEL ? kLabelTileWords + 1 : kLabelTileWords) && word < words;
-        const long long at = live ? word : 0;
-        unsigned long long m[kLevelMasks];
-#pragma unroll
-        for (int k = 0; k < kLevelMasks; ++k) m[k] = levels.mask[k][at];
-        const unsigned long long vis = d_visited[at];
-        const unsigned long long nev = (!RELABEL && d_never) ? d_never[at] : 0ull;
-        unsigned long long pl[4] = {0ull, 0ull, 0ull, 0ull}, later = 0ull;
-#pragma unroll
-        for (int k = kLevelMasks - 1; k >= 0; --k) {
-            const unsigned long long own = (k < valid ? m[k] : 0ull) & ~later;
-            later |= own;
-#pragma unroll
-            for (int p = 0; p < 4; ++p)
-                if (((k + 1) >> p) & 1) pl[p] |= own;
-        }
-        const unsigned long long kept = vis & ~nev & ~later;
-#pragma unroll
-        for (int p = 0; p < 4; ++p) {
-            if ((kCodeWorkLabel >> p) & 1u) pl[p] |= kept;
-            if (!live) pl[p] = 0ull;
-        }
-        planes[tier][2 * col] = LabelPlanes{static_cast<unsigned>(pl[0]), static_cast<unsigned>(pl[1]), static_cast<unsigned>(pl[2]), static_cast<unsigned>(pl[3])};
-        planes[tier][2 * col + 1] = LabelPlanes{static_cast<unsigned>(pl[0] >> 32), static_cast<unsigned>(pl[1] >> 32), static_cast<unsigned>(pl[2] >> 32),
-                                                static_cast<unsigned>(pl[3] >> 32)};
-    }
-    if (RELABEL && t < kLabelTileWords) {
-        const unsigned e_lo = static_cast<unsigned>(tile_edge), h_lo = static_cast<unsigned>(tile_hub);
-        const unsigned x1 = static_cast<unsigned>(map.hubs) + tile_base1;
-        s_tier[0][2 * t] = make_uint2(e_lo, x1);
-        s_tier[0][2 * t + 1] = make_uint2(static_cast<unsigned>(tile_edge >> 32), x1 + __popc(e_lo));
-        s_tier[1][2 * t] = make_uint2(h_lo, tile_base0);
-        s_tier[1][2 * t + 1] = make_uint2(static_cast<unsigned>(tile_hub >> 32), tile_base0 + __popc(h_lo));
-    }
-    __syncthreads();
     const int sh = (t & 15) * 4;
     const int half = sh >> 5, s5 = sh & 31;
     const unsigned below = (1u << s5) - 1u;
@@ -459,6 +492,103 @@
         }
     }
 }
+
+template <typename VertexId, bool RELABEL, bool PRED>
+__global__ __launch_bounds__(256) void TiledLabelsKernel(LevelMaskList<VertexId> levels, const unsigned long long *d_visited,
+                                                         const unsigned long long *d_never, graphio::RelabelView map, long long nodes,
+                                                         VertexId src, const VertexId *d_work_labels, const VertexId *d_work_preds,
+                                                         const VertexId *d_old_of_new, VertexId *d_labels, VertexId *d_preds)
+{
+    __shared__ TiledLabelsShared lds;
+    const long long w0 = static_cast<long long>(blockIdx.x) * kLabelTileWords;
+    long long xw1, xwh;
+    TiledLabelsRuns<RELABEL>(map, w0, xw1, xwh);
+    int valid = levels.count;
+    if (levels.d_gate) {
+        const int go = levels.d_gate[0], filled = levels.d_gate[1];
+        if (go == 0) return;
+        valid = levels.chain_first + filled;
+    }
+    const int t = threadIdx.x;
+    TiledLabelsLoads loads;
+    TiledLabelsLoad<VertexId, RELABEL>(loads, levels, d_visited, d_never, map, nodes, t, w0, xw1, xwh);
+    TiledLabelsFold<VertexId, RELABEL>(loads, levels, map, lds, t, valid);
+    __syncthreads();
+    TiledLabelsStore<VertexId, RELABEL, PRED>(map, nodes, src, d_work_labels, d_work_preds, d_old_of_new, d_labels, d_preds, lds, t, w0, xw1, xwh);
+}
+
+template <typename VertexId, bool RELABEL, bool PRED>
+struct TiledLabelRole {
+    static constexpr bool ENABLED = true;
+    static constexpr int QUARTERS = 4;
+    static constexpr size_t LDS_BYTES = sizeof(TiledLabelsShared) * QUARTERS * 2;
+    struct Args {
+        LevelMaskList<VertexId> levels;
+        const unsigned long long *d_visited, *d_never;
+        graphio::RelabelView map;
+        long long nodes;
+        VertexId src;
+        const VertexId *d_work_labels, *d_work_preds, *d_old_of_new;
+        VertexId *d_labels, *d_preds;
+    };
+
+    static __device__ __forceinline__ void Run(const Args &a, unsigned char *lds_bytes, const unsigned block, const unsigned blocks, const int filled)
+    {
+        TiledLabelsShared *lds = reinterpret_cast<TiledLabelsShared *>(lds_bytes);
+        const int quarter = static_cast<int>(threadIdx.x) >> 8, t = static_cast<int>(threadIdx.x) & 255;
+        const int valid = a.levels.chain_first + filled;
+        const long long words = (a.nodes + 63) / 64;
+        const long long tiles = (words + kLabelTileWords - 1) / kLabelTileWords;
+        auto tile_of = [&](long long group) -> long long {
+            const long long tile = group * QUARTERS + quarter;
+            return (group * QUARTERS < tiles && tile < tiles) ? tile : -1;
+        };
+        long long group = block;
+        long long tile = tile_of(group), next_tile = tile_of(group + blocks);
+        long long xw1 = 0, xwh = 0, next_xw1 = 0, next_xwh = 0;
+        TiledLabelsLoads loads;
+        loads.live = false;
+        if (tile >= 0) TiledLabelsRuns<RELABEL>(a.map, tile * kLabelTileWords, xw1, xwh);
+        if (next_tile >= 0) TiledLabelsRuns<RELABEL>(a.map, next_tile * kLabelTileWords, next_xw1, next_xwh);
+        if (tile >= 0) TiledLabelsLoad<VertexId, RELABEL>(loads, a.levels, a.d_visited, a.d_never, a.map, a.nodes, t, tile * kLabelTileWords, xw1, xwh);
+        int turn = 0;
+        for (; group * QUARTERS < tiles; group += blocks, turn ^= 1) {
+            TiledLabelsShared &set = lds[quarter * 2 + turn];
+            if (tile >= 0) TiledLabelsFold<VertexId, RELABEL>(loads, a.levels, a.map, set, t, valid);
+            util::LdsBarrier();
+            const long long after_next = tile_of(group + 2 * static_cast<long long>(blocks));
+            long long an_xw1 = 0, an_xwh = 0;
+            if (next_tile >= 0)
+                TiledLabelsLoad<VertexId, RELABEL>(loads, a.levels, a.d_visited, a.d_never, a.map, a.nodes, t, next_tile * kLabelTileWords, next_xw1,
+                                                   next_xwh);
+            if (after_next >= 0) TiledLabelsRuns<RELABEL>(a.map, after_next * kLabelTileWords, an_xw1, an_xwh);
+            if (tile >= 0)
+                TiledLabelsStore<VertexId, RELABEL, PRED>(a.map, a.nodes, a.src, a.d_work_labels, a.d_work_preds, a.d_old_of_new, a.d_labels, a.d_preds,
+                                                          set, t, tile * kLabelTileWords, xw1, xwh);
+            tile = next_tile;
+            xw1 = next_xw1;
+            xwh = next_xwh;
+            next_tile = after_next;
+            next_xw1 = an_xw1;
+            next_xwh = an_xwh;
+        }
+    }
+
+    static __device__ __forceinline__ void Patch(const Args &a, const int x, const int label)
+    {
+        if (x < 0 || x >= a.nodes) return;
+        if (RELABEL) {
+            const VertexId v = a.d_old_of_new[x];
+            a.d_labels[v] = label;
+            if (PRED) {
+                const VertexId pr = __hip_atomic_load(a.d_work_preds + x, __ATOMIC_RELAXED, __HIP_MEMORY_SCOPE_AGENT);
+                a.d_preds[v] = pr >= 0 ? a.d_old_of_new[pr] : pr;
+            }
+        } else {
+            a.d_labels[x] = label;
+        }
+    }
+};
 
 template <typename VertexId, typename SizeT>
 struct SearchGraph {
@@ -599,6 +729,7 @@
                     if (ds->d_frontier_mask[i]) util::GRError(hipFree(ds->d_frontier_mask[i]), "BFSProblem hipFree d_frontier_mask failed", __FILE__, __LINE__);
                 if (ds->d_snapshot) util::GRError(hipFree(ds->d_snapshot), "BFSProblem hipFree d_snapshot failed", __FILE__, __LINE__);
                 if (ds->d_fresh) util::GRError(hipFree(ds->d_fresh), "BFSProblem hipFree d_fresh failed", __FILE__, __LINE__);
+                ReleaseClosingLog();
                 delete ds;
             }
             delete[] data_slices;
@@ -633,7 +764,7 @@
         if (active == 1) UseNumbering(0);
         numbering[1].Release();
         GR_CHECK(relabelled.Build(this->nodes, this->edges, numbering[0].d_row_offsets, numbering[0].d_column_indices, hubs < 0 ? 0 : hubs,
-                                  MARK_PREDECESSORS, stream),
+                                  true, stream),
                  "BFSProblem relabel build failed");
         numbering[1].d_row_offsets = relabelled.d_row_offsets;
         numbering[1].d_column_indices = relabelled.d_cols;
@@ -698,6 +829,7 @@
         GR_CHECK(numbering[0].Build(static_cast<long long>(this->nodes), MaskWords(), this->graph_slices[0]->stream),
                  "BFSProblem static search state failed");
         UseNumbering(0);
+        GR_CHECK(EnsureClosingLog(), "BFSProblem closing log allocation failed");
 
         if (alpha_ > 0) alpha = alpha_;
         if (beta_ > 0) beta = beta_;
@@ -1016,6 +1148,99 @@
         return rc;
     }
 
+    int closing_fused = 0;
+    int closing_workgroups = 0;
+    long long closing_log_limit = 0;
+    long long closing_fused_launches = 0;
+    int2 *d_closing_log = nullptr;
+    unsigned closing_log_capacity = 0;
+    unsigned *d_closing_words = nullptr;
+    unsigned long long *d_closing_counters = nullptr;
+
+    unsigned ClosingLogWanted() const
+    {
+        long long want = closing_log_limit > 0 ? closing_log_limit : 4ll * persistent_edge_limit;
+        if (closing_log_limit <= 0 && want > static_cast<long long>(this->nodes)) want = this->nodes;
+        if (want < 1) want = 1;
+        if (want > (1ll << 30)) want = 1ll << 30;
+        return static_cast<unsigned>(want);
+    }
+    void ReleaseClosingLog()
+    {
+        if (d_closing_log) util::GRError(hipFree(d_closing_log), "BFSProblem hipFree closing log failed", __FILE__, __LINE__);
+        if (d_closing_words) util::GRError(hipFree(d_closing_words), "BFSProblem hipFree closing words failed", __FILE__, __LINE__);
+        if (d_closing_counters) util::GRError(hipFree(d_closing_counters), "BFSProblem hipFree closing counters failed", __FILE__, __LINE__);
+        d_closing_log = nullptr;
+        d_closing_words = nullptr;
+        d_closing_counters = nullptr;
+        closing_log_capacity = 0;
+    }
+    hipError_t EnsureClosingLog()
+    {
+        hipError_t retval = hipSuccess;
+        const unsigned want = ClosingLogWanted();
+        if (!d_closing_words) {
+            GR_CHECK(hipMalloc(&d_closing_words, sizeof(unsigned) * 4), "BFSProblem hipMalloc closing words failed");
+            GR_CHECK(hipMalloc(&d_closing_counters, sizeof(unsigned long long) * 2), "BFSProblem hipMalloc closing counters failed");
+            GR_CHECK(hipMemset(d_closing_words, 0, sizeof(unsigned) * 4), "BFSProblem hipMemset closing words failed");
+            GR_CHECK(hipMemset(d_closing_counters, 0, sizeof(unsigned long long) * 2), "BFSProblem hipMemset closing counters failed");
+            GR_CHECK(hipDeviceSynchronize(), "BFSProblem sync failed");
+        }
+        if (d_closing_log && closing_log_capacity == want) return retval;
+        if (d_closing_log) {
+            GR_CHECK(hipStreamSynchronize(this->graph_slices[0]->stream), "BFSProblem sync failed");
+            GR_CHECK(hipFree(d_closing_log), "BFSProblem hipFree closing log failed");
+            d_closing_log = nullptr;
+        }
+        GR_CHECK(hipMalloc(&d_closing_log, sizeof(int2) * static_cast<size_t>(want)), "BFSProblem hipMalloc closing log failed");
+        closing_log_capacity = want;
+        return retval;
+    }
+    bool ClosingFusable(int chain_count) const
+    {
+        return closing_fused != 0 && label_pass != 0 && labels_deferred && speculative_emit && chain_closing &&
+               level_masks.count + chain_count <= kLevelMasks;
+    }
+    template <bool RELABEL, bool PRED>
+    void FillLabelRole(typename TiledLabelRole<VertexId, RELABEL, PRED>::Args &a, const int *chain_masks, const VertexId *chain_labels,
+                       int chain_count)
+    {
+        DataSlice *ds = data_slices[0];
+        const unsigned long long *vis = reinterpret_cast<const unsigned long long *>(ds->d_visited_mask);
+        LevelMaskList<VertexId> list = level_masks;
+        list.chain_first = list.count;
+        for (int k = 0; k < chain_count; ++k) {
+            list.mask[list.count] = reinterpret_cast<const unsigned long long *>(ds->d_frontier_mask[chain_masks[k]]);
+            list.label[list.count] = chain_labels[k];
+            ++list.count;
+        }
+        for (int k = list.count; k < kLevelMasks; ++k) {
+            list.mask[k] = list.count > 0 ? list.mask[0] : vis;
+            list.label[k] = -1;
+        }
+        a.levels = list;
+        a.d_visited = vis;
+        a.d_never = reinterpret_cast<const unsigned long long *>(ds->d_never_mask);
+        a.nodes = static_cast<long long>(this->nodes);
+        if (RELABEL) {
+            a.map = relabelled.View();
+            a.src = (caller_source >= 0 && caller_source < this->nodes) ? caller_source : static_cast<VertexId>(-1);
+            a.d_work_labels = d_work_labels;
+            a.d_work_preds = d_work_preds;
+            a.d_old_of_new = relabelled.d_old_of_new;
+            a.d_labels = d_out_labels;
+            a.d_preds = d_out_preds;
+        } else {
+            a.map = graphio::RelabelView();
+            a.src = (source >= 0 && source < this->nodes) ? source : static_cast<VertexId>(-1);
+            a.d_work_labels = ds->d_labels;
+            a.d_work_preds = nullptr;
+            a.d_old_of_new = nullptr;
+            a.d_labels = ds->d_labels;
+            a.d_preds = nullptr;
+        }
+    }
+
     util::WorkProgress *arm_progress = nullptr;
     util::WorkProgress *armed_progress = nullptr;
 
diff --git a/gunrockinst_amd/csrc/gunrock/oprtr/advance/kernel.hpp b/gunrockinst_amd/csrc/gunrock/oprtr/advance/kernel.hpp
--- a/gunrockinst_amd/csrc/gunrock/oprtr/advance/kernel.hpp
+++ b/gunrockinst_amd/csrc/gunrock/oprtr/advance/kernel.hpp
@@ -49,6 +49,7 @@
     unsigned long long *d_duty = nullptr;
     const void *d_value_to_reduce = nullptr;
     void *d_reduced_value = nullptr;
+    DiscoveryLog log;
 };
 
 template <bool FRESH, typename T>
@@ -257,7 +258,7 @@
         }
         if constexpr (!COUNT_ONLY) {
             if (pending > KernelPolicy::STAGE_CAPACITY - TILE) {
-                if (OUT_WITH_DEGREES) Writer::template Flush<true>(sh.writer, pending, a.out, a.d_tail_out, a.d_overflow, a.d_row_offsets);
+                if (OUT_WITH_DEGREES) Writer::template Flush<true>(sh.writer, pending, a.out, a.d_tail_out, a.d_overflow, a.d_row_offsets, a.log);
                 else Writer::FlushIds(sh.writer, pending, a.out.v, a.out.capacity, a.d_tail_out, a.d_overflow);
             }
         }
@@ -676,7 +677,7 @@
     int *d_timeout;
 };
 
-__device__ __forceinline__ bool GridBarrier(const GridBarrierState &b, unsigned &epoch)
+__device__ __forceinline__ bool GridBarrier(const GridBarrierState &b, unsigned &epoch, const unsigned participants)
 {
     __shared__ int s_ok;
     asm volatile("s_waitcnt vmcnt(0)" ::: "memory");
@@ -685,7 +686,7 @@
         __builtin_amdgcn_fence(__ATOMIC_RELEASE, "agent");
         asm volatile("s_waitcnt vmcnt(0)" ::: "memory");
         epoch += 1;
-        const unsigned target = epoch * gridDim.x;
+        const unsigned target = epoch * participants;
         __hip_atomic_fetch_add(b.d_counter, 1u, __ATOMIC_RELAXED, __HIP_MEMORY_SCOPE_AGENT);
         int ok = 1;
         unsigned spins = 0;
@@ -718,13 +719,14 @@
 
 template <typename KernelPolicy, typename ProblemData, typename Functor>
 __device__ __forceinline__ void PersistentLevelsBody(const PersistentArgs<typename ProblemData::VertexId, typename ProblemData::SizeT> &p,
-                                                     typename ProblemData::DataSlice &slice, const long long first_iteration)
+                                                     typename ProblemData::DataSlice &slice, const long long first_iteration,
+                                                     AdvanceShared<KernelPolicy, typename ProblemData::VertexId, typename ProblemData::SizeT> &sh,
+                                                     const unsigned workgroups, const DiscoveryLog &log)
 {
     typedef typename ProblemData::VertexId VertexId;
     typedef typename ProblemData::SizeT SizeT;
     typedef AdvanceShared<KernelPolicy, VertexId, SizeT> Shared;
     typedef typename Shared::Writer Writer;
-    __shared__ Shared sh;
     const TailArgs<VertexId, SizeT> &t = p.t;
 
     Writer::Init(sh.writer);
@@ -735,7 +737,7 @@
     long long unexplored = p.unexplored_edges;
     int done = 0;
     unsigned epoch = 0;
-    bool solo = (gridDim.x == 1);
+    bool solo = (workgroups == 1);
     unsigned long long sum_len = 0, sum_edges = 0;
     for (;;) {
         if (threadIdx.x == 0) {
@@ -753,7 +755,7 @@
         if (!solo && edges <= p.solo_edges) {
             if (blockIdx.x != 0) return;
             solo = true;
-        } else if (solo && gridDim.x > 1 && edges > p.solo_edges)
+        } else if (solo && workgroups > 1 && edges > p.solo_edges)
             break;
 
         AdvanceArgs<VertexId, SizeT> a;
@@ -766,10 +768,12 @@
         a.d_tail_out = t.d_tail + ((iteration + 1) & 3);
         a.d_tail_clear = nullptr;
         a.d_overflow = t.d_overflow;
+        a.log = log;
+        a.log.tag = static_cast<int>(iteration) + 1;
         slice.iteration = static_cast<VertexId>(iteration);
 
         const long long tiles = (static_cast<long long>(edges) + KernelPolicy::TILE - 1) / KernelPolicy::TILE;
-        const long long per_block = solo ? tiles : (tiles + gridDim.x - 1) / gridDim.x;
+        const long long per_block = solo ? tiles : (tiles + workgroups - 1) / workgroups;
         const long long tile_begin = static_cast<long long>(blockIdx.x) * per_block;
         const long long tile_end = (tile_begin + per_block < tiles) ? tile_begin + per_block : tiles;
         if (tile_begin < tile_end) {
@@ -777,12 +781,12 @@
             ExpandTiles<KernelPolicy, ProblemData, Functor, true, true>(a, slice, tile_begin, tile_end, sh, accepted, tile_tag);
             const int rest = Writer::Count(sh.writer);
             __syncthreads();
-            Writer::template Flush<true>(sh.writer, rest, a.out, a.d_tail_out, a.d_overflow, a.d_row_offsets);
+            Writer::template Flush<true>(sh.writer, rest, a.out, a.d_tail_out, a.d_overflow, a.d_row_offsets, a.log);
         }
         if (solo) {
             asm volatile("s_waitcnt vmcnt(0)" ::: "memory");
             __syncthreads();
-        } else if (!GridBarrier(p.barrier, epoch))
+        } else if (!GridBarrier(p.barrier, epoch, workgroups))
             break;
         selector ^= 1;
         ++iteration;
@@ -802,14 +806,34 @@
 __global__ __launch_bounds__(KernelPolicy::THREADS) void PersistentLevelsKernel(
     PersistentArgs<typename ProblemData::VertexId, typename ProblemData::SizeT> p, typename ProblemData::DataSlice slice)
 {
-    PersistentLevelsBody<KernelPolicy, ProblemData, Functor>(p, slice, p.t.first_iteration);
-}
-
-template <typename KernelPolicy, typename ProblemData, typename Functor>
+    __shared__ AdvanceShared<KernelPolicy, typename ProblemData::VertexId, typename ProblemData::SizeT> sh;
+    PersistentLevelsBody<KernelPolicy, ProblemData, Functor>(p, slice, p.t.first_iteration, sh, gridDim.x, DiscoveryLog());
+}
+
+struct NoLabelRole {
+    static constexpr bool ENABLED = false;
+    static constexpr size_t LDS_BYTES = 0;
+    struct Args {};
+};
+
+struct ClosingFuse {
+    unsigned closing_workgroups = 0;
+    DiscoveryLog log;
+    unsigned *d_arrived = nullptr;
+    int *d_log_overflow = nullptr;
+    unsigned long long *d_counters = nullptr;
+};
+
+template <typename KernelPolicy, typename ProblemData, typename Functor, typename LabelRole = NoLabelRole>
 __global__ __launch_bounds__(KernelPolicy::THREADS) void ChainedPersistentLevelsKernel(
     PersistentArgs<typename ProblemData::VertexId, typename ProblemData::SizeT> p, typename ProblemData::DataSlice slice,
-    SweepChain chain, int sweeps, long long first_level, const int *d_queue_invalid, int *d_gate)
-{
+    SweepChain chain, int sweeps, long long first_level, const int *d_queue_invalid, int *d_gate, typename LabelRole::Args labels,
+    ClosingFuse fuse)
+{
+    typedef AdvanceShared<KernelPolicy, typename ProblemData::VertexId, typename ProblemData::SizeT> Shared;
+    constexpr size_t LDS_BYTES = sizeof(Shared) > LabelRole::LDS_BYTES ? sizeof(Shared) : LabelRole::LDS_BYTES;
+    __shared__ __attribute__((aligned(16))) unsigned char lds[LDS_BYTES];
+    Shared &sh = *reinterpret_cast<Shared *>(lds);
     const ChainEnd end = ChainOutcome(chain, sweeps, util::LaneId());
     const bool run = end.action == kSweepSwitch && end.end >= 2 && end.prev_action == kSweepSparseEmit && *d_queue_invalid == 0;
     if (blockIdx.x == 0 && threadIdx.x == 0) {
@@ -819,10 +843,51 @@
             *p.t.d_levels_done = 0;
             p.t.d_level_sums[0] = 0ull;
             p.t.d_level_sums[1] = 0ull;
+            if constexpr (LabelRole::ENABLED) *fuse.d_log_overflow = 0;
         }
     }
     if (!run) return;
-    PersistentLevelsBody<KernelPolicy, ProblemData, Functor>(p, slice, first_level + (end.end - 1));
+    if constexpr (!LabelRole::ENABLED) {
+        PersistentLevelsBody<KernelPolicy, ProblemData, Functor>(p, slice, first_level + (end.end - 1), sh, gridDim.x, DiscoveryLog());
+    } else {
+        if (blockIdx.x < fuse.closing_workgroups)
+            PersistentLevelsBody<KernelPolicy, ProblemData, Functor>(p, slice, first_level + (end.end - 1), sh, fuse.closing_workgroups, fuse.log);
+        else
+            LabelRole::Run(labels, lds, blockIdx.x - fuse.closing_workgroups, gridDim.x - fuse.closing_workgroups, end.end - 1);
+        asm volatile("s_waitcnt vmcnt(0)" ::: "memory");
+        __syncthreads();
+        int *s_last = reinterpret_cast<int *>(lds);
+        if (threadIdx.x == 0) {
+            __builtin_amdgcn_fence(__ATOMIC_RELEASE, "agent");
+            asm volatile("s_waitcnt vmcnt(0)" ::: "memory");
+            const unsigned before = __hip_atomic_fetch_add(fuse.d_arrived, 1u, __ATOMIC_RELAXED, __HIP_MEMORY_SCOPE_AGENT);
+            const int last = before + 1u == gridDim.x ? 1 : 0;
+            if (last) {
+                __builtin_amdgcn_fence(__ATOMIC_ACQUIRE, "agent");
+                asm volatile("s_waitcnt vmcnt(0)" ::: "memory");
+            }
+            *s_last = last;
+        }
+        __syncthreads();
+        if (*s_last == 0) return;
+        const unsigned count = __hip_atomic_load(fuse.log.d_count, __ATOMIC_RELAXED, __HIP_MEMORY_SCOPE_AGENT);
+        const bool overflow = count > fuse.log.capacity;
+        if (!overflow) {
+            for (unsigned i = threadIdx.x; i < count; i += KernelPolicy::THREADS) {
+                int2 e;
+                e.x = __hip_atomic_load(&fuse.log.d_entries[i].x, __ATOMIC_RELAXED, __HIP_MEMORY_SCOPE_AGENT);
+                e.y = __hip_atomic_load(&fuse.log.d_entries[i].y, __ATOMIC_RELAXED, __HIP_MEMORY_SCOPE_AGENT);
+                LabelRole::Patch(labels, e.x, e.y);
+            }
+        }
+        if (threadIdx.x == 0) {
+            *fuse.d_log_overflow = overflow ? 1 : 0;
+            if (overflow) fuse.d_counters[1] += 1ull;
+            else fuse.d_counters[0] += count;
+            __hip_atomic_store(fuse.log.d_count, 0u, __ATOMIC_RELAXED, __HIP_MEMORY_SCOPE_AGENT);
+            __hip_atomic_store(fuse.d_arrived, 0u, __ATOMIC_RELAXED, __HIP_MEMORY_SCOPE_AGENT);
+        }
+    }
 }
 
 template <typename KernelPolicy, typename ProblemData, typename Functor>
@@ -856,8 +921,28 @@
     if (grid > cu_count) grid = cu_count;
     if (grid < 1) grid = 1;
     hipLaunchKernelGGL((ChainedPersistentLevelsKernel<KernelPolicy, ProblemData, Functor>), dim3(grid), dim3(KernelPolicy::THREADS), 0, stream, args,
-                       slice, chain, sweeps, first_level, d_queue_invalid, d_gate);
+                       slice, chain, sweeps, first_level, d_queue_invalid, d_gate, NoLabelRole::Args(), ClosingFuse());
     return util::GRError("advance::ChainedPersistentLevelsKernel launch failed", __FILE__, __LINE__);
+}
+
+constexpr int kClosingWorkgroups = 64;
+
+template <typename KernelPolicy, typename ProblemData, typename Functor, typename LabelRole>
+hipError_t LaunchChainedClosingFused(const PersistentArgs<typename ProblemData::VertexId, typename ProblemData::SizeT> &args,
+                                     const typename ProblemData::DataSlice &slice, int cu_count, const SweepChain &chain, int sweeps,
+                                     long long first_level, const int *d_queue_invalid, int *d_gate, const typename LabelRole::Args &labels,
+                                     ClosingFuse fuse, hipStream_t stream, bool &fused, int closing_workgroups = kClosingWorkgroups)
+{
+    int grid = util::ResidentGrid(ChainedPersistentLevelsKernel<KernelPolicy, ProblemData, Functor, LabelRole>, KernelPolicy::THREADS);
+    if (grid > cu_count) grid = cu_count;
+    fused = grid >= 2;
+    if (!fused) return hipSuccess;
+    if (closing_workgroups < 1) closing_workgroups = kClosingWorkgroups;
+    if (closing_workgroups > grid - 1) closing_workgroups = grid - 1;
+    fuse.closing_workgroups = static_cast<unsigned>(closing_workgroups);
+    hipLaunchKernelGGL((ChainedPersistentLevelsKernel<KernelPolicy, ProblemData, Functor, LabelRole>), dim3(grid), dim3(KernelPolicy::THREADS), 0,
+                       stream, args, slice, chain, sweeps, first_level, d_queue_invalid, d_gate, labels, fuse);
+    return util::GRError("advance::ChainedPersistentLevelsKernel (fused) launch failed", __FILE__, __LINE__);
 }
 
 template <typename KernelPolicy, typename ProblemData, typename Functor>
diff --git a/gunrockinst_amd/csrc/gunrock/oprtr/frontier_writer.hpp b/gunrockinst_amd/csrc/gunrock/oprtr/frontier_writer.hpp
--- a/gunrockinst_amd/csrc/gunrock/oprtr/frontier_writer.hpp
+++ b/gunrockinst_amd/csrc/gunrock/oprtr/frontier_writer.hpp
@@ -7,6 +7,13 @@
 
 namespace gunrock {
 namespace oprtr {
+
+struct DiscoveryLog {
+    int2 *d_entries = nullptr;
+    unsigned *d_count = nullptr;
+    unsigned capacity = 0;
+    int tag = 0;
+};
 
 template <int THREADS, int CAPACITY, typename VertexId, typename SizeT>
 struct FrontierWriter {
@@ -19,6 +26,7 @@
         typename Scan::Storage scan;
         unsigned long long base;
         int count;
+        unsigned log_base;
     };
 
     static __device__ __forceinline__ void Init(Storage &st)
@@ -54,9 +62,11 @@
     static __device__ __forceinline__ void Flush(Storage &st, const int n,
                                                  const util::Frontier<VertexId, SizeT> &out,
                                                  unsigned long long *d_tail, int *d_overflow,
-                                                 const SizeT *__restrict__ d_row_offsets)
+                                                 const SizeT *__restrict__ d_row_offsets, const DiscoveryLog log = DiscoveryLog())
     {
         if (n == 0) return;
+        if (log.d_entries && threadIdx.x == THREADS - 1)
+            st.log_base = __hip_atomic_fetch_add(log.d_count, static_cast<unsigned>(n), __ATOMIC_RELAXED, __HIP_MEMORY_SCOPE_AGENT);
 
         VertexId v[PER_THREAD];
         SizeT rs[PER_THREAD];
@@ -82,6 +92,14 @@
         }
         __syncthreads();
         const unsigned long long block_base = st.base;
+        if (log.d_entries) {
+            const unsigned log_base = st.log_base;
+#pragma unroll
+            for (int j = 0; j < PER_THREAD; ++j) {
+                const int i = j * THREADS + threadIdx.x;
+                if (i < n && log_base + static_cast<unsigned>(i) < log.capacity) log.d_entries[log_base + i] = make_int2(static_cast<int>(v[j]), log.tag);
+            }
+        }
         if (static_cast<unsigned long long>(util::TailCount(block_base)) + util::TailCount(total) >
             static_cast<unsigned long long>(out.capacity)) {
             if (threadIdx.x == 0) *d_overflow = 1;
diff --git a/gunrockinst_amd/csrc/lib/bfs_app.hip b/gunrockinst_amd/csrc/lib/bfs_app.hip
--- a/gunrockinst_amd/csrc/lib/bfs_app.hip
+++ b/gunrockinst_amd/csrc/lib/bfs_app.hip
@@ -42,6 +42,7 @@
     virtual void DeviceResults(int **labels, int **preds) = 0;
     virtual void BuildRelabelled(bool on) = 0;
     virtual long long MaskFlushes() = 0;
+    virtual hipError_t ClosingInfo(long long &fused_launches, long long &patched_vertices, long long &log_overflows) = 0;
     virtual void RelabelInfo(long long &hubs, long long &with_edges, int &threshold, float &build_ms, long long &bytes) = 0;
 };
 
@@ -123,6 +124,14 @@
         else if (key == "chain_closing") problem.chain_closing = value != 0.0;
         else if (key == "label_pass") problem.label_pass = value != 0.0 ? 1 : 0;
         else if (key == "walk_queue") problem.walk_queue = value != 0.0 ? 1 : 0;
+        else if (key == "closing_fused") problem.closing_fused = value != 0.0 ? 1 : 0;
+        else if (key == "closing_workgroups") {
+            if (value < 0.0) return 2;
+            problem.closing_workgroups = static_cast<int>(value);
+        } else if (key == "closing_log_limit") {
+            if (value < 0.0) return 2;
+            problem.closing_log_limit = static_cast<long long>(value);
+        }
         else if (key == "relabel") {
             if (value > 0.0 && !problem.HasRelabelled()) return 2;
             problem.relabel = value > 0.0 ? 1 : (value < 0.0 ? -1 : 0);
@@ -139,6 +148,19 @@
     }
     void BuildRelabelled(bool on) override { problem.build_relabelled = on; }
     long long MaskFlushes() override { return problem.mask_flushes; }
+    hipError_t ClosingInfo(long long &fused_launches, long long &patched_vertices, long long &log_overflows) override
+    {
+        hipError_t retval = hipSuccess;
+        fused_launches = problem.closing_fused_launches;
+        patched_vertices = log_overflows = 0;
+        if (!problem.d_closing_counters) return retval;
+        unsigned long long counters[2] = {0ull, 0ull};
+        GR_CHECK(hipStreamSynchronize(problem.graph_slices[0]->stream), "BFS closing info sync failed");
+        GR_CHECK(hipMemcpy(counters, problem.d_closing_counters, sizeof(counters), hipMemcpyDeviceToHost), "BFS closing info read failed");
+        patched_vertices = static_cast<long long>(counters[0]);
+        log_overflows = static_cast<long long>(counters[1]);
+        return retval;
+    }
     void RelabelInfo(long long &hubs, long long &with_edges, int &threshold, float &build_ms, long long &bytes) override
     {
         const bool ready = problem.HasRelabelled();
@@ -387,6 +409,17 @@
     if (!p || !p->runner || !flushes) return -1;
     *flushes = p->runner->MaskFlushes();
     return 0;
+}
+
+int grx_bfs_closing_info(grx_bfs *p, long long *fused_launches, long long *patched_vertices, long long *log_overflows)
+{
+    if (!p || !p->runner) return -1;
+    long long f = 0, v = 0, o = 0;
+    const hipError_t rc = p->runner->ClosingInfo(f, v, o);
+    if (fused_launches) *fused_launches = f;
+    if (patched_vertices) *patched_vertices = v;
+    if (log_overflows) *log_overflows = o;
+    return static_cast<int>(rc);
 }
 
 int grx_bfs_relabel_info(grx_bfs *p, long long *hubs, long long *with_edges, int *threshold, float *build_ms, long long *bytes)
diff --git a/include/gunrock/gunrock_mi355x.h b/include/gunrock/gunrock_mi355x.h
--- a/include/gunrock/gunrock_mi355x.h
+++ b/include/gunrock/gunrock_mi355x.h
@@ -53,6 +53,7 @@
 int grx_bfs_set_label_deferral(grx_bfs *p, int enabled, int mask_limit);
 int grx_bfs_set_option(grx_bfs *p, const char *name, double value);
 int grx_bfs_mask_flushes(grx_bfs *p, long long *flushes);
+int grx_bfs_closing_info(grx_bfs *p, long long *fused_launches, long long *patched_vertices, long long *log_overflows);
 int grx_bfs_relabel_info(grx_bfs *p, long long *hubs, long long *with_edges, int *threshold, float *build_ms, long long *bytes);
 int grx_bfs_set_head_pass(grx_bfs *p, int min_edges, int max_edges);
 int grx_bfs_reset(grx_bfs *p, int src, double queue_sizing);
```

Result: slower. 997,300 MTEPS (-1.9%).
